# succinctlabs/sp1

Hardware: NVIDIA H100
Metric: riscv_cycles_proven_per_second_core (higher is better)
Workload: dtype u32 KoalaBear (Montgomery) / ext4

## Files before the change

### include/sp1b200.h

```cpp
#ifndef SP1B200_H
#define SP1B200_H
#include <stdint.h>
#include <stddef.h>

#ifdef __cplusplus
extern "C" {
#endif

typedef struct sp1b200_ctx sp1b200_ctx;
typedef const char* sp1b200_err;

typedef struct sp1b200_params {
    uint32_t log_stacking_height;
    uint32_t max_log_row_count;
    uint32_t log_blowup;
    uint32_t num_queries;
    uint32_t pow_bits;
    uint32_t batch_pow_bits;
    uint32_t gkr_pow_bits;
    uint32_t grind_mode;
} sp1b200_params;

#define SP1B200_CHALLENGER_WORDS 34
#define SP1B200_DIGEST_WORDS 8

sp1b200_err sp1b200_ctx_create(int device, const sp1b200_params* params, sp1b200_ctx** out);
void sp1b200_ctx_destroy(sp1b200_ctx* ctx);
sp1b200_err sp1b200_ctx_sync(sp1b200_ctx* ctx);
void sp1b200_default_core_params(sp1b200_params* out);
const char* sp1b200_version(void);
void* sp1b200_ctx_stream(sp1b200_ctx* ctx);
sp1b200_err sp1b200_malloc(sp1b200_ctx* ctx, size_t bytes, void** d_out);
sp1b200_err sp1b200_free(sp1b200_ctx* ctx, void* d_ptr);
sp1b200_err sp1b200_memcpy_h2d(sp1b200_ctx* ctx, void* d_dst, const void* h_src, size_t bytes);
sp1b200_err sp1b200_memcpy_d2h(sp1b200_ctx* ctx, void* h_dst, const void* d_src, size_t bytes);
sp1b200_err sp1b200_pack_row_major(sp1b200_ctx* ctx, const uint32_t* rows_any, uint32_t n_tables, const uint64_t* rows,
                                   const uint64_t* cols, uint32_t* d_dense_out);
sp1b200_err sp1b200_upload_begin(sp1b200_ctx* ctx, const uint32_t* h_src, uint64_t n_words, int slot, uint32_t** d_out);
uint64_t sp1b200_launch_count(sp1b200_ctx* ctx);
float sp1b200_last_phase_ms(sp1b200_ctx* ctx, const char* phase);


sp1b200_err sp1b200_poseidon2_permute(sp1b200_ctx* ctx, uint32_t* states_any, uint64_t n);

sp1b200_err sp1b200_rs_encode(sp1b200_ctx* ctx, const uint32_t* msg_any, uint64_t ncols, uint32_t log_h,
                              uint32_t log_blowup, uint32_t* out_any);

sp1b200_err sp1b200_merkle_commit(sp1b200_ctx* ctx, const uint32_t* mat_any, uint64_t width, uint32_t log_h,
                                  uint32_t* d_layers_out, uint32_t* h_root8, uint32_t* h_commit8);

sp1b200_err sp1b200_grind(sp1b200_ctx* ctx, uint32_t* h_state34, uint32_t bits, uint32_t* h_witness);

void sp1b200_challenger_init(uint32_t* h_state34);
void sp1b200_challenger_observe(uint32_t* h_state34, const uint32_t* h_vals, uint64_t n);
void sp1b200_challenger_sample(uint32_t* h_state34, uint32_t* h_out, uint64_t n);
uint32_t sp1b200_challenger_sample_bits(uint32_t* h_state34, uint32_t bits);
int sp1b200_challenger_check_witness(uint32_t* h_state34, uint32_t bits, uint32_t witness);


typedef struct sp1b200_commit sp1b200_commit;

sp1b200_err sp1b200_stacked_commit(sp1b200_ctx* ctx, const uint32_t* dense_any, uint64_t ncols, int keep_codeword,
                                   uint32_t* h_commit8, sp1b200_commit** out);
void sp1b200_commit_free(sp1b200_ctx* ctx, sp1b200_commit* c);

sp1b200_err sp1b200_stacked_prove(sp1b200_ctx* ctx, sp1b200_commit* const* rounds, uint32_t n_rounds,
                                  const uint32_t* h_point, uint32_t n_point, const uint32_t* h_replay_witnesses,
                                  uint32_t* h_challenger34, uint32_t* h_proof, uint64_t proof_cap_words,
                                  uint64_t* h_proof_words);


typedef struct sp1b200_jagged_round sp1b200_jagged_round;

sp1b200_err sp1b200_jagged_commit(sp1b200_ctx* ctx, const uint32_t* dense_any, uint32_t n_tables, const uint64_t* h_rows,
                                  const uint64_t* h_cols, int keep_codeword, uint32_t* h_commit8, sp1b200_jagged_round** out);
void sp1b200_jagged_round_free(sp1b200_ctx* ctx, sp1b200_jagged_round* round);

sp1b200_err sp1b200_jagged_column_claims(sp1b200_ctx* ctx, const sp1b200_jagged_round* round, const uint32_t* h_z_row,
                                         uint32_t* h_out);

sp1b200_err sp1b200_jagged_prove(sp1b200_ctx* ctx, sp1b200_jagged_round* const* rounds, uint32_t n_rounds,
                                 const uint32_t* h_z_row, const uint32_t* h_claims, const uint32_t* h_replay_witnesses,
                                 uint32_t* h_challenger34, uint32_t* h_proof, uint64_t proof_cap_words,
                                 uint64_t* h_proof_words);


typedef struct sp1b200_machine sp1b200_machine;

sp1b200_err sp1b200_machine_create(sp1b200_ctx* ctx, const uint32_t* h_blob, uint64_t n_words, sp1b200_machine** out);
void sp1b200_machine_free(sp1b200_ctx* ctx, sp1b200_machine* machine);
uint32_t sp1b200_machine_num_chips(const sp1b200_machine* machine);
uint32_t sp1b200_machine_chip_regs(const sp1b200_machine* machine, uint32_t chip);

sp1b200_err sp1b200_zerocheck(sp1b200_ctx* ctx, const sp1b200_machine* machine, const uint64_t* h_heights,
                              const uint32_t* const* d_main, const uint32_t* const* d_prep, const uint32_t* h_public_values,
                              uint32_t n_public_values, const uint32_t* h_gkr_point, const uint32_t* h_alpha,
                              const uint32_t* h_gamma, const uint32_t* h_claims, uint32_t* h_challenger34, uint32_t* h_out,
                              uint64_t out_cap_words, uint64_t* h_out_words);



sp1b200_err sp1b200_logup_gkr(sp1b200_ctx* ctx, const sp1b200_machine* machine, const uint64_t* h_heights,
                              const uint32_t* const* d_main, const uint32_t* const* d_prep, const uint32_t* h_replay_witness,
                              uint32_t* h_challenger34, uint32_t* h_out, uint64_t out_cap_words, uint64_t* h_out_words);


sp1b200_err sp1b200_prove_shard(sp1b200_ctx* ctx, const sp1b200_machine* machine, sp1b200_jagged_round* prep_round,
                                const uint32_t* main_dense_any, const uint64_t* h_heights, const char* const* chip_names,
                                const uint32_t* h_public_values, uint32_t n_public_values, const uint32_t* h_replay_witnesses,
                                uint32_t* h_challenger34, uint32_t* h_proof, uint64_t proof_cap_words, uint64_t* h_proof_words);

sp1b200_err sp1b200_setup_and_prove_shard(sp1b200_ctx* ctx, const sp1b200_machine* machine, const uint32_t* prep_dense_any, uint32_t n_prep,
                                          const uint64_t* h_prep_rows, const uint64_t* h_prep_cols, const uint32_t* h_vk_tail,
                                          uint32_t n_vk_tail, const uint32_t* main_dense_any, const uint64_t* h_heights,
                                          const char* const* chip_names, const uint32_t* h_public_values, uint32_t n_public_values,
                                          const uint32_t* h_replay_witnesses, uint32_t* h_challenger34, uint32_t* h_prep_commit8,
                                          sp1b200_jagged_round** prep_round_out, uint32_t* h_proof, uint64_t proof_cap_words,
                                          uint64_t* h_proof_words);


sp1b200_err sp1b200_debug_constraints(sp1b200_ctx* ctx, const sp1b200_machine* machine, sp1b200_jagged_round* prep_round,
                                      const uint32_t* main_dense_any, const uint64_t* h_heights, const uint32_t* h_public_values,
                                      uint32_t n_public_values, uint32_t max_rows_per_chip, uint32_t* h_out, uint64_t out_cap_words,
                                      uint64_t* h_out_words);

sp1b200_err sp1b200_debug_interactions(sp1b200_ctx* ctx, const sp1b200_machine* machine, sp1b200_jagged_round* prep_round,
                                       const uint32_t* main_dense_any, const uint64_t* h_heights, uint32_t max_keys, uint32_t* h_out,
                                       uint64_t out_cap_words, uint64_t* h_out_words);


sp1b200_err sp1b200_shard_proof_to_bincode(const sp1b200_params* params, uint32_t n_chips, const char* const* chip_names,
                                           const uint64_t* h_heights, const uint32_t* h_main_w, const uint32_t* h_prep_w,
                                           const uint32_t* h_proof, uint64_t n_words, uint8_t* h_out, uint64_t cap_bytes,
                                           uint64_t* h_out_bytes);
sp1b200_err sp1b200_shard_proof_from_bincode(const sp1b200_params* params, uint32_t n_chips, const char* const* chip_names,
                                             const uint32_t* h_main_w, const uint32_t* h_prep_w, const uint8_t* h_bytes, uint64_t n_bytes,
                                             uint64_t* h_heights_out, uint32_t* h_proof, uint64_t cap_words, uint64_t* h_words);

#define SP1B200_VERDICT_ACCEPT 0u
#define SP1B200_VERDICT_POW 1u
#define SP1B200_VERDICT_INVALID_SHAPE 2u
#define SP1B200_VERDICT_ZERO_DENOMINATOR 3u
#define SP1B200_VERDICT_CUMULATIVE_SUM_MISMATCH 4u
#define SP1B200_VERDICT_INVALID_SHAPE_ROUNDS 5u
#define SP1B200_VERDICT_INCONSISTENT_SUMCHECK_CLAIM 6u
#define SP1B200_VERDICT_SUMCHECK_PROOF_SHAPE 7u
#define SP1B200_VERDICT_SUMCHECK_CLAIMED_SUM 8u
#define SP1B200_VERDICT_SUMCHECK_ROUND 9u
#define SP1B200_VERDICT_SUMCHECK_POINT 10u
#define SP1B200_VERDICT_SUMCHECK_EVAL 11u
#define SP1B200_VERDICT_INCONSISTENT_EVALUATION 12u
#define SP1B200_VERDICT_LAST_LAYER_DIMENSION 13u
#define SP1B200_VERDICT_TRACE_POINT_MISMATCH 14u
#define SP1B200_VERDICT_INVALID_SHAPE_OPENINGS 15u
#define SP1B200_VERDICT_NUMERATOR_EVALUATION 16u
#define SP1B200_VERDICT_DENOMINATOR_EVALUATION 17u
#define SP1B200_VERDICT_OPENING_SHAPE 18u
#define SP1B200_VERDICT_HEIGHT_BITS 19u
#define SP1B200_VERDICT_HEIGHT_TOO_LARGE 20u
#define SP1B200_VERDICT_CONSTRAINTS_EVAL 21u
#define SP1B200_VERDICT_CONSTRAINTS_CLAIMED_SUM 22u
#define SP1B200_VERDICT_INCORRECT_SHAPE 23u
#define SP1B200_VERDICT_INCORRECT_TABLE_SIZES 24u
#define SP1B200_VERDICT_AREA_OUT_OF_BOUNDS 25u
#define SP1B200_VERDICT_DUMMY_TABLES 26u
#define SP1B200_VERDICT_SUMCHECK_CLAIM_MISMATCH 27u
#define SP1B200_VERDICT_MONOTONICITY 28u
#define SP1B200_VERDICT_JAGGED_EVALUATION 29u
#define SP1B200_VERDICT_JAGGED_EVAL_PROOF 30u
#define SP1B200_VERDICT_STACKING 31u
#define SP1B200_VERDICT_BATCH_POW 32u
#define SP1B200_VERDICT_FRI_LENGTH 33u
#define SP1B200_VERDICT_BASEFOLD_SUMCHECK 34u
#define SP1B200_VERDICT_TWO_ADICITY 35u
#define SP1B200_VERDICT_TCS_COMPONENT 36u
#define SP1B200_VERDICT_QUERY_VALUE 37u
#define SP1B200_VERDICT_TCS_QUERY 38u
#define SP1B200_VERDICT_QUERY_FINAL_POLY 39u
#define SP1B200_VERDICT_SUMCHECK_FINAL_POLY 40u
#define SP1B200_VERDICT_PREPROCESSED_WIDTHS 41u
#define SP1B200_VERDICT_CHIP_TABLES 42u
sp1b200_err sp1b200_verify_shard(sp1b200_ctx* ctx, const sp1b200_machine* machine, const uint32_t* h_prep_commit8,
                                 const uint64_t* h_heights, const char* const* chip_names, const uint32_t* h_proof, uint64_t n_words,
                                 uint32_t* h_challenger34, uint32_t* h_verdict);
const char* sp1b200_verdict_name(uint32_t verdict);

#define SP1B200_VERDICT_EMPTY_PROOF 43u
#define SP1B200_VERDICT_TOO_MANY_SHARDS 44u
#define SP1B200_VERDICT_INVALID_SHARD_PROOF 45u
#define SP1B200_VERDICT_PV_LENGTH 46u
#define SP1B200_VERDICT_PV_FIRST_SHARD_MULTIPLE 47u
#define SP1B200_VERDICT_PV_FIRST_SHARD_NOT_BOOLEAN 48u
#define SP1B200_VERDICT_PV_FIRST_SHARD_NOT_SET 49u
#define SP1B200_VERDICT_PV_INITIAL_TIMESTAMP 50u
#define SP1B200_VERDICT_PV_TIMESTAMP_UNCHANGED 51u
#define SP1B200_VERDICT_PV_TIMESTAMP_CHANGED 52u
#define SP1B200_VERDICT_PV_PC_START_VK 53u
#define SP1B200_VERDICT_PV_PC_START_PREV 54u
#define SP1B200_VERDICT_PV_PC_NON_EXECUTION 55u
#define SP1B200_VERDICT_PV_NOT_HALTED 56u
#define SP1B200_VERDICT_PV_PREV_EXIT_CODE 57u
#define SP1B200_VERDICT_PV_EXIT_CODE_NON_EXECUTION 58u
#define SP1B200_VERDICT_PV_EXIT_CODE_CHANGED 59u
#define SP1B200_VERDICT_PV_PROOF_NONCE 60u
#define SP1B200_VERDICT_PV_INIT_ADDR 61u
#define SP1B200_VERDICT_PV_FINALIZE_ADDR 62u
#define SP1B200_VERDICT_PV_INIT_PAGE_IDX 63u
#define SP1B200_VERDICT_PV_FINALIZE_PAGE_IDX 64u
#define SP1B200_VERDICT_PV_UNTRUSTED_PROGRAMS 65u
#define SP1B200_VERDICT_PV_NEVER_INITIALIZED 66u
#define SP1B200_VERDICT_PV_NEVER_FINALIZED 67u
#define SP1B200_VERDICT_PV_COMMITTED_VALUE_DIGEST 68u
#define SP1B200_VERDICT_PV_DEFERRED_PROOFS_DIGEST 69u
#define SP1B200_VERDICT_PV_COMMIT_SYSCALL 70u
#define SP1B200_VERDICT_PV_COMMIT_DEFERRED_SYSCALL 71u
#define SP1B200_VERDICT_PV_COMMIT_NEVER_CALLED 72u
#define SP1B200_VERDICT_PV_COMMIT_DEFERRED_NEVER_CALLED 73u
#define SP1B200_VERDICT_PV_GLOBAL_CUMULATIVE_SUM 74u
#define SP1B200_VERDICT_PV_EXCEPTIONAL_ADDITION 75u
#define SP1B200_VERDICT_CORE_COUNT 76u
sp1b200_err sp1b200_verify_core_proof(sp1b200_ctx* ctx, const sp1b200_machine* machine, const uint32_t* h_prep_commit8,
                                      const uint32_t* h_vk_tail, uint32_t n_vk_tail, uint32_t n_shards, const uint64_t* h_heights,
                                      const char* const* chip_names, const uint32_t* const* h_proofs, const uint64_t* h_n_words,
                                      uint32_t host_threads, uint32_t* h_final_challengers, uint32_t* h_verdict, uint32_t* h_shard,
                                      uint32_t* h_shard_verdict);

#ifdef __cplusplus
}
#endif
#endif
```

### sp1_b200/csrc/ctx.cuh

```cuda
#pragma once
#include <cuda_runtime.h>
#include <chrono>
#include <cstdint>
#include <cstdio>
#include <map>
#include <memory>
#include <string>
#include <vector>
#include "../../include/sp1b200.h"

struct sp1b200_ctx {
    int device = 0;
    int num_sms = 132;
    cudaStream_t stream = nullptr;
    cudaMemPool_t pool = nullptr;
    sp1b200_params params{};
    uint32_t* d_TH = nullptr;
    uint32_t* d_TL = nullptr;
    uint32_t* d_T8 = nullptr;
    uint64_t launches = 0;
    bool force_generic_ntt = false;
    std::map<std::string, float> phase_ms;
    cudaEvent_t ev0 = nullptr, ev1 = nullptr;
    uint32_t* h_mail = nullptr;
    uint32_t* d_mail = nullptr;
    uint32_t* d_mail_counter = nullptr;
    uint32_t mail_seq = 0;
    cudaStream_t copy_stream = nullptr;
    uint32_t* d_slot[2] = {nullptr, nullptr};
    uint64_t slot_words[2] = {0, 0};
    cudaEvent_t slot_ready[2] = {nullptr, nullptr};
    cudaEvent_t slot_free[2] = {nullptr, nullptr};
    bool slot_pending[2] = {false, false};
    std::unique_ptr<uint32_t[]> shard_scratch;
};
constexpr size_t SP1_MAIL_HDR = 16;
constexpr size_t SP1_MAIL_WORDS = 1 << 16;

struct Mail { uint32_t* flag; uint32_t* counter; uint32_t seq; };
inline Mail sp1b200_mail_next(sp1b200_ctx* c) { return Mail{c->d_mail, c->d_mail_counter, ++c->mail_seq}; }
inline uint32_t* sp1b200_mail_dev(sp1b200_ctx* c) { return c->d_mail + SP1_MAIL_HDR; }
inline const uint32_t* sp1b200_mail_host(sp1b200_ctx* c) { return c->h_mail + SP1_MAIL_HDR; }
extern "C" sp1b200_err sp1b200_mail_wait(sp1b200_ctx* c, uint32_t seq);

sp1b200_err sp1b200_init_tables(sp1b200_ctx* ctx);
sp1b200_err sp1b200_rs_encode_device(sp1b200_ctx* ctx, const uint32_t* d_msg, uint64_t ncols, uint32_t log_h, uint32_t log_blowup,
                                     uint32_t* d_out);
sp1b200_err sp1b200_permute_device(sp1b200_ctx* ctx, uint32_t* d_states, uint64_t n);
sp1b200_err sp1b200_merkle_commit_device(sp1b200_ctx* ctx, const uint32_t* d_mat, uint64_t width, uint32_t log_h, uint32_t* d_layers,
                                         uint32_t* d_root_commit16);
sp1b200_err sp1b200_merkle_tree_from_leaves_device(sp1b200_ctx* ctx, uint32_t* d_layers, uint32_t log_h, uint32_t width,
                                                   uint32_t* d_root_commit16);
sp1b200_err sp1b200_fri_tree_device(sp1b200_ctx* ctx, const uint32_t* d_cw, uint64_t m, uint32_t* d_layers, uint32_t log_leaves,
                                    uint32_t* d_root_commit16, Mail mail);

#ifdef __CUDACC__
__device__ __forceinline__ void sp1_mail_done(const Mail& m) {
    if (!m.flag) return;
    __threadfence_system();
    __syncthreads();
    if (threadIdx.x == 0 && threadIdx.y == 0 && threadIdx.z == 0) {
        const unsigned total = gridDim.x * gridDim.y * gridDim.z;
        const unsigned prev = atomicAdd(m.counter, 1u);
        if (prev == total - 1) {
            *m.counter = 0;
            __threadfence_system();
            *reinterpret_cast<volatile uint32_t*>(m.flag) = m.seq;
        }
    }
}
#endif

const char* sp1b200_set_error(const char* fmt, ...);
const char* sp1b200_last_error();

struct Sp1DeviceGuard {
    int prev = -1;
    bool switched = false;
    explicit Sp1DeviceGuard(int dev) {
        if (dev < 0) return;
        if (cudaGetDevice(&prev) == cudaSuccess && prev != dev) switched = cudaSetDevice(dev) == cudaSuccess;
    }
    ~Sp1DeviceGuard() { if (switched) cudaSetDevice(prev); }
    Sp1DeviceGuard(const Sp1DeviceGuard&) = delete;
    Sp1DeviceGuard& operator=(const Sp1DeviceGuard&) = delete;
};
#define SP1_DEVICE_GUARD(c) Sp1DeviceGuard _sp1_device_guard((c) ? (c)->device : -1)

#define SP1_CUDA(call)                                                                            \
    do {                                                                                          \
        cudaError_t _e = (call);                                                                  \
        if (_e != cudaSuccess)                                                                    \
            return sp1b200_set_error("%s:%d: %s: %s", __FILE__, __LINE__, #call, cudaGetErrorString(_e)); \
    } while (0)

#define SP1_TRY(call)                   \
    do {                                \
        sp1b200_err _m = (call);        \
        if (_m) return _m;              \
    } while (0)

#define SP1_LAUNCH(ctx, kernel, grid, block, smem, ...)                        \
    do {                                                                       \
        kernel<<<(grid), (block), (smem), (ctx)->stream>>>(__VA_ARGS__);       \
        (ctx)->launches++;                                                     \
        SP1_CUDA(cudaGetLastError());                                          \
    } while (0)

struct PhaseTimer {
    sp1b200_ctx* ctx;
    const char* name;
    cudaEvent_t e0 = nullptr, e1 = nullptr;
    bool done = false;
    PhaseTimer(sp1b200_ctx* c, const char* n) : ctx(c), name(n) {
        cudaEventCreate(&e0); cudaEventCreate(&e1);
        cudaEventRecord(e0, c->stream);
    }
    void stop() {
        if (done) return;
        done = true;
        cudaEventRecord(e1, ctx->stream);
        cudaEventSynchronize(e1);
        float ms = 0;
        cudaEventElapsedTime(&ms, e0, e1);
        ctx->phase_ms[name] = ms;
    }
    ~PhaseTimer() { cudaEventDestroy(e0); cudaEventDestroy(e1); }
};

struct HostAccum {
    sp1b200_ctx* ctx; const char* name; double ms = 0;
    HostAccum(sp1b200_ctx* c, const char* n) : ctx(c), name(n) {}
    ~HostAccum() { ctx->phase_ms[name] = (float)ms; }
};
struct HostSpan {
    HostAccum& a; std::chrono::steady_clock::time_point t0;
    explicit HostSpan(HostAccum& acc) : a(acc), t0(std::chrono::steady_clock::now()) {}
    ~HostSpan() { a.ms += std::chrono::duration<double, std::milli>(std::chrono::steady_clock::now() - t0).count(); }
};

struct DevBuf {
    sp1b200_ctx* ctx = nullptr;
    void* d = nullptr;
    void* host = nullptr;
    size_t bytes = 0;
    bool owned = false;
    sp1b200_err in(sp1b200_ctx* c, const void* any, size_t nbytes);
    sp1b200_err out(sp1b200_ctx* c, void* any, size_t nbytes);
    sp1b200_err finish();
    ~DevBuf();
};

bool sp1b200_is_device_ptr(const void* p);
extern "C" int sp1b200_upload_acquire(sp1b200_ctx* c, const void* d_ptr);
extern "C" void sp1b200_upload_release(sp1b200_ctx* c, int slot);
```

### sp1_b200/csrc/hostcheck.cu

```cuda
#include "poseidon2.cuh"
#include "rs_twiddles.cuh"
#include "debug_fp.cuh"
#include "hostfield.hpp"
#include "septic.hpp"
#include "zc_lower.hpp"
#include <cstring>
#include <type_traits>

extern "C" {
void sp1b200_hostcheck_permute(uint32_t* states, uint64_t n) {
    for (uint64_t i = 0; i < n; i++) {
        uint32_t s[16];
        for (int k = 0; k < 16; k++) s[k] = states[i * 16 + k];
        p2::permute(s);
        for (int k = 0; k < 16; k++) states[i * 16 + k] = s[k];
    }
}
int sp1b200_hostcheck_permute_mode(uint32_t* states, uint64_t n, int mode) {
    for (uint64_t i = 0; i < n; i++) {
        uint32_t s[16];
        for (int k = 0; k < 16; k++) s[k] = states[i * 16 + k];
        switch (mode) {
#define P2_CASE(M) case M: p2::permute_m<M>(s); break;
            P2_CASE(0) P2_CASE(1) P2_CASE(2) P2_CASE(3) P2_CASE(4) P2_CASE(5) P2_CASE(6) P2_CASE(7)
            P2_CASE(8) P2_CASE(9) P2_CASE(10) P2_CASE(11) P2_CASE(12) P2_CASE(13) P2_CASE(14) P2_CASE(15)
            P2_CASE(19) P2_CASE(21) P2_CASE(23)
#undef P2_CASE
            case -1: p2::permute_r1(s); break;
            default: return 0;
        }
        for (int k = 0; k < 16; k++) states[i * 16 + k] = s[k];
    }
    return 1;
}
void sp1b200_hostcheck_ext_mul(const uint32_t* a, const uint32_t* b, uint32_t* out, uint64_t n) {
    for (uint64_t i = 0; i < n; i++) {
        kb::Ext x{{a[4 * i], a[4 * i + 1], a[4 * i + 2], a[4 * i + 3]}}, y{{b[4 * i], b[4 * i + 1], b[4 * i + 2], b[4 * i + 3]}};
        kb::Ext r = kb::ext_mul(x, y);
        for (int k = 0; k < 4; k++) out[4 * i + k] = r.c[k];
    }
}
void sp1b200_hostcheck_ext_inv(const uint32_t* a, uint32_t* out, uint64_t n) {
    for (uint64_t i = 0; i < n; i++) {
        kb::Ext x{{a[4 * i], a[4 * i + 1], a[4 * i + 2], a[4 * i + 3]}};
        kb::Ext r = kb::ext_inv(x);
        for (int k = 0; k < 4; k++) out[4 * i + k] = r.c[k];
    }
}
uint32_t sp1b200_hostcheck_rs_tw8(uint32_t* out) {
    for (uint32_t i = 0; i < rs_tw::WORDS; i++) out[i] = rs_tw::word(i / 8, (int)(i % 8));
    return rs_tw::WORDS;
}
void sp1b200_hostcheck_field(const uint32_t* a, const uint32_t* b, uint32_t* add, uint32_t* sub, uint32_t* mul, uint64_t n) {
    for (uint64_t i = 0; i < n; i++) { add[i] = kb::add(a[i], b[i]); sub[i] = kb::sub(a[i], b[i]); mul[i] = kb::mul(a[i], b[i]); }
}

int sp1b200_hostcheck_zc_lower(const uint32_t* chip, const uint32_t* main_row, const uint32_t* prep_row, const uint32_t* pv,
                               const uint32_t* alpha_pows, uint32_t window, uint32_t* out, uint32_t* n_lowered) {
    using hf::E4;
    const uint32_t* b = chip;
    HostProg hp;
    b += 3;
    const uint32_t n_regs = *b++;
    const uint32_t ni = *b++, nl = *b++, nc = *b++, np = *b++, na = *b++;
    hp.instrs.resize(ni); memcpy(hp.instrs.data(), b, ni * 8); b += 2 * ni;
    hp.leaves.resize(nl); memcpy(hp.leaves.data(), b, nl * 8); b += 2 * nl;
    hp.consts.assign(b, b + nc); b += nc;
    hp.publics.assign(b, b + np); b += np;
    hp.assert_regs.assign(b, b + na); b += na;
    hp.assert_alphas.assign(b, b + na); b += na;
    auto leaf = [&](const LeafRef& l) { return l.source == LEAF_MAIN ? main_row[l.col] : prep_row[l.col]; };
    {
        std::vector<uint32_t> regs(n_regs ? n_regs : 1, 0);
        for (const DagInstr& in : hp.instrs) {
            switch (in.opcode) {
                case BC_LOAD_LEAF: regs[in.out] = leaf(hp.leaves[in.a]); break;
                case BC_LOAD_CONST: regs[in.out] = hp.consts[in.a]; break;
                case BC_LOAD_PUBLIC: regs[in.out] = pv[hp.publics[in.a]]; break;
                case BC_ADD_F: regs[in.out] = hf::add(regs[in.a], regs[in.b]); break;
                case BC_SUB_F: regs[in.out] = hf::sub(regs[in.a], regs[in.b]); break;
                case BC_MUL_F: regs[in.out] = hf::mul(regs[in.a], regs[in.b]); break;
                case BC_NEG_F: regs[in.out] = hf::neg(regs[in.a]); break;
            }
        }
        E4 acc;
        for (size_t k = 0; k < hp.assert_regs.size(); k++) acc = acc + E4::load(alpha_pows + 4 * hp.assert_alphas[k]) * regs[hp.assert_regs[k]];
        acc.store(out);
    }
    auto run = [&](const ZcLowered& Lw) {
        std::vector<uint32_t> rf(Lw.n_regs, 0);
        E4 a;
        for (const ZcInstr& in : Lw.instrs) {
            switch (in.op) {
                case ZC_LOAD_MAIN: rf[in.out] = main_row[(uint32_t)in.a | ((uint32_t)in.b << 16)]; break;
                case ZC_LOAD_PREP: rf[in.out] = prep_row[(uint32_t)in.a | ((uint32_t)in.b << 16)]; break;
                case ZC_CONST: rf[in.out] = hp.consts[in.a]; break;
                case ZC_PUBLIC: rf[in.out] = pv[hp.publics[in.a]]; break;
                case ZC_ADD: { uint32_t x = rf[in.a], y = rf[in.b]; rf[in.out] = hf::add(x, y); break; }
                case ZC_SUB: { uint32_t x = rf[in.a], y = rf[in.b]; rf[in.out] = hf::sub(x, y); break; }
                case ZC_MUL: { uint32_t x = rf[in.a], y = rf[in.b]; rf[in.out] = hf::mul(x, y); break; }
                case ZC_NEG: rf[in.out] = hf::neg(rf[in.a]); break;
                case ZC_ASSERT: a = a + E4::load(alpha_pows + 4 * in.b) * rf[in.a]; break;
            }
        }
        return a;
    };
    ZcLowered L = zc_lower(hp, window);
    if (!L.error.empty()) return -1;
    if (n_lowered) *n_lowered = (uint32_t)L.instrs.size();
    E4 acc = run(L);
    {
        const size_t na = hp.assert_regs.size();
        const size_t np_ = std::max<size_t>(1, std::min<size_t>(16, na / 4));
        E4 sum;
        for (size_t q = 0; q < np_; q++) {
            ZcLowered P = zc_lower(hp, window, na * q / np_, na * (q + 1) / np_);
            if (!P.error.empty() || P.n_regs > L.n_regs + 8) return -1;
            sum = sum + run(P);
        }
        sum.store(out + 8);
    }
    acc.store(out + 4);
    return (int)L.n_regs;
}

uint64_t sp1b200_hostcheck_fingerprint(uint32_t kind, uint32_t n_values, const uint32_t* values) {
    return dbgfp::fingerprint(kind, n_values, values);
}

void sp1b200_hostcheck_e4(const uint32_t* a, const uint32_t* b, uint32_t* mul_out, uint32_t* inv_out, uint64_t n) {
    using hf::E4;
    for (uint64_t i = 0; i < n; i++) {
        (E4::load(a + 4 * i) * E4::load(b + 4 * i)).store(mul_out + 4 * i);
        hf::inv(E4::load(a + 4 * i)).store(inv_out + 4 * i);
    }
}
int sp1b200_hostcheck_interpolate(const uint32_t* xs, const uint32_t* ys, uint32_t n, uint32_t* coeffs_out) {
    using hf::E4;
    auto go = [&](auto tag) {
        constexpr int N = decltype(tag)::value;
        E4 x[N], L[N][N], c[N];
        for (int i = 0; i < N; i++) x[i] = E4::load(xs + 4 * i);
        hf::lagrange_basis<N>(x, L);
        for (int k = 0; k < N; k++) for (int i = 0; i < N; i++) c[k] = c[k] + L[i][k] * E4::load(ys + 4 * i);
        for (int k = 0; k < N; k++) c[k].store(coeffs_out + 4 * k);
    };
    if (n == 3) go(std::integral_constant<int, 3>{});
    else if (n == 4) go(std::integral_constant<int, 4>{});
    else if (n == 5) go(std::integral_constant<int, 5>{});
    else return -1;
    return 0;
}

void sp1b200_hostcheck_septic(const uint32_t* a, const uint32_t* b, uint32_t* mul_out, uint32_t* inv_out, uint64_t n) {
    for (uint64_t i = 0; i < n; i++) {
        const sep::E7 x = sep::E7::load(a + 7 * i), y = sep::E7::load(b + 7 * i);
        (x * y).store(mul_out + 7 * i);
        sep::inv(x).store(inv_out + 7 * i);
    }
}
void sp1b200_hostcheck_septic_curve_add(const uint32_t* p, const uint32_t* q, uint32_t* out, uint32_t* ok, uint64_t n) {
    for (uint64_t i = 0; i < n; i++) {
        const sep::Point a{sep::E7::load(p + 14 * i), sep::E7::load(p + 14 * i + 7)}, b{sep::E7::load(q + 14 * i), sep::E7::load(q + 14 * i + 7)};
        sep::Point r{};
        ok[i] = sep::add_incomplete(a, b, r);
        r.x.store(out + 14 * i); r.y.store(out + 14 * i + 7);
    }
}
int sp1b200_hostcheck_septic_digest_add(const uint32_t* a, const uint32_t* b, uint32_t* out) {
    const sep::Point x{sep::E7::load(a), sep::E7::load(a + 7)}, y{sep::E7::load(b), sep::E7::load(b + 7)};
    sep::Point r{};
    if (!sep::digest_add(x, y, r)) return 0;
    r.x.store(out); r.y.store(out + 7);
    return 1;
}
void sp1b200_hostcheck_septic_constants(uint32_t* out42) {
    const sep::Point pts[3] = {sep::digest_zero(), sep::digest_start(), sep::dummy_point()};
    for (int i = 0; i < 3; i++) { pts[i].x.store(out42 + 14 * i); pts[i].y.store(out42 + 14 * i + 7); }
}
}
```

### sp1_b200/csrc/machine.cuh

```cuda
#pragma once
#include "hostfield.hpp"
#include <algorithm>
#include <cstdint>
#include <type_traits>
#include <utility>
#include <vector>

struct DagInstr { uint8_t opcode, pad; uint16_t out, a, b; };
struct LeafRef { uint8_t source, pad; uint16_t pad2; uint32_t col; };
static_assert(sizeof(DagInstr) == 8 && sizeof(LeafRef) == 8, "bytecode layout must match sequential.cuh");
enum : uint8_t { BC_LOAD_LEAF = 0, BC_LOAD_CONST = 1, BC_LOAD_PUBLIC = 2, BC_ADD_F = 3, BC_SUB_F = 4, BC_MUL_F = 5, BC_NEG_F = 6 };
enum : uint8_t { LEAF_PREP = 2, LEAF_MAIN = 4 };

struct ZcInstr;
struct ChipProg {
    const DagInstr* instrs; const LeafRef* leaves; const uint32_t* consts; const uint32_t* publics;
    const uint32_t* assert_regs; const uint32_t* assert_alphas;
    uint32_t n_instrs, n_asserts, n_regs, main_w, prep_w, n_constraints;
    const ZcInstr* zc; uint32_t n_zc, zc_regs;
};
struct HostProg {
    std::vector<DagInstr> instrs; std::vector<LeafRef> leaves; std::vector<uint32_t> consts, publics, assert_regs, assert_alphas;
    std::vector<std::pair<uint32_t, uint32_t>> zc_pieces;
};

template <class R, class Leaf>
hf::E4 host_eval_constraints(const HostProg& p, uint32_t n_regs, const uint32_t* pv, const std::vector<hf::E4>& powers, Leaf leaf) {
    const auto base = [](uint32_t x) { if constexpr (std::is_same<R, hf::E4>::value) return hf::E4::from_base(x); else return x; };
    std::vector<R> regs(std::max<uint32_t>(n_regs, 1));
    for (const DagInstr& in : p.instrs) {
        switch (in.opcode) {
            case BC_LOAD_LEAF: regs[in.out] = leaf(p.leaves[in.a]); break;
            case BC_LOAD_CONST: regs[in.out] = base(p.consts[in.a]); break;
            case BC_LOAD_PUBLIC: regs[in.out] = base(pv[p.publics[in.a]]); break;
            case BC_ADD_F: regs[in.out] = hf::add(regs[in.a], regs[in.b]); break;
            case BC_SUB_F: regs[in.out] = hf::sub(regs[in.a], regs[in.b]); break;
            case BC_MUL_F: regs[in.out] = hf::mul(regs[in.a], regs[in.b]); break;
            case BC_NEG_F: regs[in.out] = hf::neg(regs[in.a]); break;
        }
    }
    hf::E4 acc;
    for (size_t i = 0; i < p.assert_regs.size(); i++) acc = acc + powers[p.assert_alphas[i]] * regs[p.assert_regs[i]];
    return acc;
}

struct TermDev { uint32_t source, col, weight; };
struct VColDev { uint32_t term_start, n_terms, constant; };
struct InterDev { uint32_t is_send, arg_index, n_values, vcol_start; };
struct HostInteractions {
    std::vector<std::vector<InterDev>> per_chip;
    std::vector<VColDev> vcols;
    std::vector<TermDev> terms;
};

void sp1b200_free_interactions(void* p);

struct sp1b200_machine {
    sp1b200_machine() = default;
    sp1b200_machine(const sp1b200_machine&) = delete;
    sp1b200_machine& operator=(const sp1b200_machine&) = delete;
    ~sp1b200_machine();
    std::vector<ChipProg> chips;
    std::vector<HostProg> host;
    uint32_t* d_arena = nullptr;
    void* d_zc_arena = nullptr;
    ChipProg* d_chips = nullptr;
    void* interactions = nullptr;
};

void* sp1b200_parse_interactions(const uint32_t* b, const uint32_t* end, size_t n_chips, const uint32_t* widths);

typedef const char* sp1b200_err;
struct sp1b200_ctx;
sp1b200_err sp1b200_debug_constraints_device(sp1b200_ctx* ctx, const sp1b200_machine* m, const uint64_t* h_heights, const uint32_t* const* d_main,
                                             const uint32_t* const* d_prep, const uint32_t* h_pv, uint32_t n_pv, uint32_t max_rows,
                                             std::vector<uint32_t>& words);
sp1b200_err sp1b200_debug_interactions_device(sp1b200_ctx* ctx, const sp1b200_machine* m, const uint64_t* h_heights, const uint32_t* const* d_main,
                                              const uint32_t* const* d_prep, uint32_t max_keys, std::vector<uint32_t>& words);
```

### sp1_b200/csrc/zerocheck.cu

```cuda
#include "ctx.cuh"
#include "challenger.cuh"
#include "hostfield.hpp"
#include "kb31.cuh"
#include <algorithm>
#include <memory>
#include <vector>

#include "machine.cuh"
#include "zc_lower.hpp"
#include "sumcheck.cuh"

namespace {

using kb::Ext;
using hf::E4;

constexpr int ZC_BLOCK = 128;
constexpr int ZC_LOCAL_REGS = 128;
constexpr int ZC_GLOBAL_REGS = 1024;
constexpr unsigned ZC_GLOBAL_MAXB = 132 * 2;
constexpr size_t ZC_MAX_PIECES = 16;

inline int zc_tier(uint32_t regs) {
    constexpr uint32_t TIER_REGS[3] = {8, 16, 32};
    for (int t = 0; t < 3; t++) if (regs <= TIER_REGS[t]) return t;
    return regs <= (uint32_t)ZC_LOCAL_REGS ? 3 : 4;
}

template <class K> struct Ops;
template <> struct Ops<uint32_t> {
    static __device__ __forceinline__ uint32_t zero() { return 0; }
    static __device__ __forceinline__ uint32_t from_base(uint32_t x) { return x; }
    static __device__ __forceinline__ uint32_t add(uint32_t a, uint32_t b) { return kb::add(a, b); }
    static __device__ __forceinline__ uint32_t sub(uint32_t a, uint32_t b) { return kb::sub(a, b); }
    static __device__ __forceinline__ uint32_t mul(uint32_t a, uint32_t b) { return kb::mul(a, b); }
    static __device__ __forceinline__ uint32_t load(const uint32_t* p, uint64_t i) { return __ldg(p + i); }
    static __device__ __forceinline__ Ext scale(const Ext& e, uint32_t k) { return kb::ext_mul_base(e, k); }
};
template <> struct Ops<Ext> {
    static __device__ __forceinline__ Ext zero() { return kb::ext_zero(); }
    static __device__ __forceinline__ Ext from_base(uint32_t x) { return kb::ext_from_base(x); }
    static __device__ __forceinline__ Ext add(const Ext& a, const Ext& b) { return kb::ext_add(a, b); }
    static __device__ __forceinline__ Ext sub(const Ext& a, const Ext& b) { return kb::ext_sub(a, b); }
    static __device__ __forceinline__ Ext mul(const Ext& a, const Ext& b) { return kb::ext_mul(a, b); }
    static __device__ __forceinline__ Ext load(const Ext* p, uint64_t i) { return kb::ext_load(reinterpret_cast<const uint32_t*>(p + i)); }
    static __device__ __forceinline__ Ext scale(const Ext& e, const Ext& k) { return kb::ext_mul(e, k); }
};

struct ZcJob {
    const void* main; const void* prep; const uint32_t* alpha_pows; uint64_t h;
    uint32_t blk_start, nblk, chip, columns;
    uint32_t zc_begin, zc_end;
    const void* batch;
};
static_assert(sizeof(ZcJob) == 64, "ZcJob layout");
struct ZcFixJob {
    const void* main; const void* prep; uint32_t* out; uint64_t h;
    uint32_t main_w, prep_w, blk_start, pad;
};

template <class J>
__device__ __forceinline__ int find_job(const J* __restrict__ jobs, int n, uint32_t blk) {
    int lo = 0, hi = n - 1;
    while (lo < hi) {
        int mid = (lo + hi + 1) >> 1;
        if (jobs[mid].blk_start <= blk) lo = mid; else hi = mid - 1;
    }
    return lo;
}

enum { RF_SMEM = 0, RF_LOCAL = 1, RF_GLOBAL = 2 };
template <class K, int RF, int NODES = 3> struct RegFile;
template <class K, int NODES> struct RegFile<K, RF_SMEM, NODES> {
    K* base;
    __device__ __forceinline__ RegFile(unsigned char* smem, void*, uint32_t) : base(reinterpret_cast<K*>(smem) + threadIdx.x) {}
    __device__ __forceinline__ K get(uint32_t r, int n) const { return base[(r * NODES + n) * ZC_BLOCK]; }
    __device__ __forceinline__ void set(uint32_t r, int n, const K& v) { base[(r * NODES + n) * ZC_BLOCK] = v; }
};
template <class K, int NODES> struct RegFile<K, RF_LOCAL, NODES> {
    K regs[ZC_LOCAL_REGS * NODES];
    __device__ __forceinline__ RegFile(unsigned char*, void*, uint32_t) {}
    __device__ __forceinline__ K get(uint32_t r, int n) const { return regs[r * NODES + n]; }
    __device__ __forceinline__ void set(uint32_t r, int n, const K& v) { regs[r * NODES + n] = v; }
};
template <class K, int NODES> struct RegFile<K, RF_GLOBAL, NODES> {
    K* base;
    __device__ __forceinline__ RegFile(unsigned char*, void* ws, uint32_t ws_regs)
        : base(static_cast<K*>(ws) + (size_t)blockIdx.x * ws_regs * NODES * ZC_BLOCK + threadIdx.x) {}
    __device__ __forceinline__ K get(uint32_t r, int n) const { return base[(size_t)(r * NODES + n) * ZC_BLOCK]; }
    __device__ __forceinline__ void set(uint32_t r, int n, const K& v) { base[(size_t)(r * NODES + n) * ZC_BLOCK] = v; }
};

template <class K, int N0>
__device__ __forceinline__ void load_nodes(const K* __restrict__ base, uint32_t col, uint64_t h, uint64_t i, K (&v)[3]) {
    using O = Ops<K>;
    const K* c = base + (uint64_t)col * h;
    const K z = O::load(c, 2 * i);
    const K o = (2 * i + 1 < h) ? O::load(c, 2 * i + 1) : O::zero();
    const K d = O::sub(o, z);
    const K d2 = O::add(d, d);
    if (N0 == 0) v[0] = z;
    v[1] = O::add(z, d2);
    v[2] = O::add(v[1], d2);
}

template <class K, int RF, bool FIRST>
__global__ void __launch_bounds__(ZC_BLOCK) zc_sum_kernel(const ZcJob* __restrict__ jobs, int n_jobs, const ChipProg* __restrict__ chips,
                                                          const uint32_t* __restrict__ pv, const uint32_t* __restrict__ gkr_pows,
                                                          const uint32_t* __restrict__ E, uint32_t* __restrict__ partial,
                                                          void* __restrict__ ws, uint32_t ws_regs) {
    using O = Ops<K>;
    constexpr int N0 = FIRST ? 1 : 0;
    extern __shared__ __align__(16) unsigned char zc_smem[];
    __shared__ uint32_t red[5][4][ZC_BLOCK / 32];
    const ZcJob job = jobs[find_job(jobs, n_jobs, blockIdx.x)];
    const ChipProg& prog = chips[job.chip];
    const K* main = static_cast<const K*>(job.main);
    const K* prep = static_cast<const K*>(job.prep);
    const uint64_t h = job.h;
    const uint64_t terms = (h + 1) / 2;
    RegFile<K, RF> rf(zc_smem, ws, ws_regs);
    Ext acc[5];
#pragma unroll
    for (int a = 0; a < 5; a++) acc[a] = kb::ext_zero();
    const ZcInstr* __restrict__ zc = prog.zc + job.zc_begin;
    const uint32_t n_zc = job.zc_end - job.zc_begin;
    for (uint64_t i = (uint64_t)(blockIdx.x - job.blk_start) * ZC_BLOCK + threadIdx.x; i < terms; i += (uint64_t)job.nblk * ZC_BLOCK) {
        const Ext e = kb::ext_load(E + 4 * i);
        Ext row[3] = {kb::ext_zero(), kb::ext_zero(), kb::ext_zero()};
        ZcInstr in = n_zc ? zc[0] : ZcInstr{};
        for (uint32_t pc = 0; pc < n_zc; pc++) {
            const ZcInstr nxt = zc[pc + 1 < n_zc ? pc + 1 : pc];
            switch (in.op) {
                case ZC_LOAD_MAIN: case ZC_LOAD_PREP: {
                    K v[3];
                    load_nodes<K, N0>(in.op == ZC_LOAD_MAIN ? main : prep, (uint32_t)in.a | ((uint32_t)in.b << 16), h, i, v);
#pragma unroll
                    for (int n = N0; n < 3; n++) rf.set(in.out, n, v[n]);
                    break;
                }
                case ZC_CONST: { const K c = O::from_base(prog.consts[in.a]);
#pragma unroll
                    for (int n = N0; n < 3; n++) rf.set(in.out, n, c);
                    break; }
                case ZC_PUBLIC: { const K c = O::from_base(pv[prog.publics[in.a]]);
#pragma unroll
                    for (int n = N0; n < 3; n++) rf.set(in.out, n, c);
                    break; }
                case ZC_ADD: {
                    K r[3];
#pragma unroll
                    for (int n = N0; n < 3; n++) r[n] = O::add(rf.get(in.a, n), rf.get(in.b, n));
#pragma unroll
                    for (int n = N0; n < 3; n++) rf.set(in.out, n, r[n]);
                    break; }
                case ZC_SUB: {
                    K r[3];
#pragma unroll
                    for (int n = N0; n < 3; n++) r[n] = O::sub(rf.get(in.a, n), rf.get(in.b, n));
#pragma unroll
                    for (int n = N0; n < 3; n++) rf.set(in.out, n, r[n]);
                    break; }
                case ZC_MUL: {
                    K r[3];
#pragma unroll
                    for (int n = N0; n < 3; n++) r[n] = O::mul(rf.get(in.a, n), rf.get(in.b, n));
#pragma unroll
                    for (int n = N0; n < 3; n++) rf.set(in.out, n, r[n]);
                    break; }
                case ZC_NEG: {
                    K r[3];
#pragma unroll
                    for (int n = N0; n < 3; n++) r[n] = O::sub(O::zero(), rf.get(in.a, n));
#pragma unroll
                    for (int n = N0; n < 3; n++) rf.set(in.out, n, r[n]);
                    break; }
                case ZC_ASSERT: {
                    const Ext al = kb::ext_load(job.alpha_pows + 4 * in.b);
#pragma unroll
                    for (int n = N0; n < 3; n++) row[n] = kb::ext_add(row[n], O::scale(al, rf.get(in.a, n)));
                    break; }
                default: __trap();
            }
            in = nxt;
        }
#pragma unroll
        for (int n = N0; n < 3; n++) acc[n] = kb::ext_add(acc[n], kb::ext_mul(row[n], e));
        if (!job.columns) continue;
        Ext s0 = kb::ext_zero(), s1 = kb::ext_zero();
        const bool has_o = 2 * i + 1 < h;
        if (job.batch) {
            const uint32_t* B = static_cast<const uint32_t*>(job.batch);
            acc[3] = kb::ext_add(acc[3], kb::ext_mul(kb::ext_load(B + 8 * i), e));
            if (has_o) acc[4] = kb::ext_add(acc[4], kb::ext_mul(kb::ext_load(B + 8 * i + 4), e));
            continue;
        }
        for (uint32_t j = 0; j < prog.main_w; j++) {
            const Ext g = kb::ext_load(gkr_pows + 4 * j);
            const K* c = main + (uint64_t)j * h;
            s0 = kb::ext_add(s0, O::scale(g, O::load(c, 2 * i)));
            if (has_o) s1 = kb::ext_add(s1, O::scale(g, O::load(c, 2 * i + 1)));
        }
        for (uint32_t j = 0; j < prog.prep_w; j++) {
            const Ext g = kb::ext_load(gkr_pows + 4 * (prog.main_w + j));
            const K* c = prep + (uint64_t)j * h;
            s0 = kb::ext_add(s0, O::scale(g, O::load(c, 2 * i)));
            if (has_o) s1 = kb::ext_add(s1, O::scale(g, O::load(c, 2 * i + 1)));
        }
        acc[3] = kb::ext_add(acc[3], kb::ext_mul(s0, e));
        acc[4] = kb::ext_add(acc[4], kb::ext_mul(s1, e));
    }
    const int lane = threadIdx.x & 31, warp = threadIdx.x >> 5;
#pragma unroll
    for (int a = 0; a < 5; a++)
#pragma unroll
        for (int l = 0; l < 4; l++) {
            uint32_t v = acc[a].c[l];
            for (int s = 16; s > 0; s >>= 1) v = kb::add(v, __shfl_down_sync(0xffffffffu, v, s));
            if (lane == 0) red[a][l][warp] = v;
        }
    __syncthreads();
    if (threadIdx.x < 36) {
        const int node = threadIdx.x / 12, slot = (threadIdx.x >> 2) % 3, l = threadIdx.x & 3;
        const int a = slot == 0 ? node : (node == 0 ? 2 + slot : -1);
        uint32_t v = 0;
        if (a >= 0)
            for (int w = 0; w < ZC_BLOCK / 32; w++) v = kb::add(v, red[a][l][w]);
        partial[(uint64_t)blockIdx.x * 36 + threadIdx.x] = v;
    }
}

__global__ void __launch_bounds__(128) zc_reduce_kernel(const ZcJob* __restrict__ jobs, const uint32_t* __restrict__ partial, uint32_t* __restrict__ out,
                                                        Mail mail) {
    const ZcJob job = jobs[blockIdx.x];
    __shared__ uint32_t red[36][4];
    const int slot = threadIdx.x >> 2, part = threadIdx.x & 3;
    for (int w = slot; w < 36; w += 32) {
        uint32_t v = 0;
        for (uint32_t b = part; b < job.nblk; b += 4) v = kb::add(v, partial[(uint64_t)(job.blk_start + b) * 36 + w]);
        red[w][part] = v;
    }
    __syncthreads();
    if (threadIdx.x < 36) {
        const uint32_t* r = red[threadIdx.x];
        out[blockIdx.x * 36 + threadIdx.x] = kb::add(kb::add(r[0], r[1]), kb::add(r[2], r[3]));
    }
    sp1_mail_done(mail);
}

template <class K>
__global__ void __launch_bounds__(256) zc_fix_kernel(const ZcFixJob* __restrict__ jobs, int n_jobs, Ext alpha) {
    using O = Ops<K>;
    const ZcFixJob job = jobs[find_job(jobs, n_jobs, blockIdx.x)];
    const uint64_t h = job.h, nh = (h + 1) / 2;
    const uint32_t bpc = (uint32_t)((nh + 255) / 256);
    const uint32_t lb = blockIdx.x - job.blk_start;
    const uint64_t j = lb / bpc;
    const uint64_t i = (uint64_t)(lb - (uint32_t)j * bpc) * 256 + threadIdx.x;
    if (i >= nh) return;
    const uint64_t t = j * nh + i;
    const K* in = j < job.main_w ? static_cast<const K*>(job.main) + j * h : static_cast<const K*>(job.prep) + (j - job.main_w) * h;
    K a = O::load(in, 2 * i);
    K b = (2 * i + 1 < h) ? O::load(in, 2 * i + 1) : O::zero();
    Ext r;
    if constexpr (sizeof(K) == 4) r = kb::ext_add(kb::ext_from_base(a), kb::ext_mul_base(alpha, kb::sub(b, a)));
    else r = kb::ext_add(a, kb::ext_mul(alpha, kb::ext_sub(b, a)));
    kb::ext_store(job.out + 4 * t, r);
}

__global__ void __launch_bounds__(256) zc_batch0_kernel(const ZcFixJob* __restrict__ jobs, int n_jobs, const uint32_t* __restrict__ gkr_pows, Ext alpha) {
    const ZcFixJob job = jobs[find_job(jobs, n_jobs, blockIdx.x)];
    const uint64_t h = job.h, nh = (h + 1) / 2;
    const uint64_t i = (uint64_t)(blockIdx.x - job.blk_start) * 256 + threadIdx.x;
    if (i >= nh) return;
    const bool has_o = 2 * i + 1 < h;
    Ext sa = kb::ext_zero(), sd = kb::ext_zero();
    const uint32_t* main = static_cast<const uint32_t*>(job.main);
    const uint32_t* prep = static_cast<const uint32_t*>(job.prep);
    for (uint32_t j = 0; j < job.main_w + job.prep_w; j++) {
        const uint32_t* c = j < job.main_w ? main + (uint64_t)j * h : prep + (uint64_t)(j - job.main_w) * h;
        const uint32_t a = __ldg(c + 2 * i), b = has_o ? __ldg(c + 2 * i + 1) : 0u;
        const Ext g = kb::ext_load(gkr_pows + 4 * j);
        sa = kb::ext_add(sa, kb::ext_mul_base(g, a));
        sd = kb::ext_add(sd, kb::ext_mul_base(g, kb::sub(b, a)));
    }
    kb::ext_store(job.out + 4 * i, kb::ext_add(sa, kb::ext_mul(alpha, sd)));
}

struct ZcDbgJob {
    const uint32_t* main; const uint32_t* prep; uint64_t h;
    const uint32_t* rows;
    uint32_t* out;
    uint32_t* count;
    uint32_t n, blk_start, nblk, chip, cwords, pad;
};
static_assert(sizeof(ZcDbgJob) == 72, "ZcDbgJob layout");

template <int RF, bool LISTED>
__global__ void __launch_bounds__(ZC_BLOCK) zc_debug_kernel(const ZcDbgJob* __restrict__ jobs, int n_jobs, const ChipProg* __restrict__ chips,
                                                            const uint32_t* __restrict__ pv, void* __restrict__ ws, uint32_t ws_regs) {
    extern __shared__ __align__(16) unsigned char zc_smem[];
    const ZcDbgJob job = jobs[find_job(jobs, n_jobs, blockIdx.x)];
    const ChipProg& prog = chips[job.chip];
    RegFile<uint32_t, RF, 1> rf(zc_smem, ws, ws_regs);
    const ZcInstr* __restrict__ zc = prog.zc;
    const uint32_t n_zc = prog.n_zc, lane = threadIdx.x & 31;
    for (uint64_t t0 = (uint64_t)(blockIdx.x - job.blk_start) * ZC_BLOCK + (threadIdx.x - lane); t0 < job.n; t0 += (uint64_t)job.nblk * ZC_BLOCK) {
        const uint64_t t = t0 + lane;
        bool fail = false;
        if (t < job.n) {
            const uint64_t row = LISTED ? job.rows[t] : t;
            for (uint32_t pc = 0; pc < n_zc; pc++) {
                const ZcInstr in = zc[pc];
                switch (in.op) {
                    case ZC_LOAD_MAIN: rf.set(in.out, 0, __ldg(job.main + (uint64_t)((uint32_t)in.a | ((uint32_t)in.b << 16)) * job.h + row)); break;
                    case ZC_LOAD_PREP: rf.set(in.out, 0, __ldg(job.prep + (uint64_t)((uint32_t)in.a | ((uint32_t)in.b << 16)) * job.h + row)); break;
                    case ZC_CONST: rf.set(in.out, 0, prog.consts[in.a]); break;
                    case ZC_PUBLIC: rf.set(in.out, 0, pv[prog.publics[in.a]]); break;
                    case ZC_ADD: rf.set(in.out, 0, kb::add(rf.get(in.a, 0), rf.get(in.b, 0))); break;
                    case ZC_SUB: rf.set(in.out, 0, kb::sub(rf.get(in.a, 0), rf.get(in.b, 0))); break;
                    case ZC_MUL: rf.set(in.out, 0, kb::mul(rf.get(in.a, 0), rf.get(in.b, 0))); break;
                    case ZC_NEG: rf.set(in.out, 0, kb::neg(rf.get(in.a, 0))); break;
                    case ZC_ASSERT:
                        if (rf.get(in.a, 0)) {
                            fail = true;
                            if (LISTED) job.out[t * job.cwords + (in.b >> 5)] |= 1u << (in.b & 31);
                        }
                        break;
                    default: __trap();
                }
            }
        }
        if (!LISTED) {
            const uint32_t bits = __ballot_sync(0xffffffffu, fail);
            if (lane == 0 && bits) { job.out[t0 >> 5] = bits; atomicAdd(job.count, (uint32_t)__popc(bits)); }
        }
    }
}

struct ZcDbgSelect { const uint32_t* bits; uint32_t* rows; uint32_t n_words, take; };
__global__ void __launch_bounds__(32) zc_debug_select_kernel(const ZcDbgSelect* __restrict__ jobs) {
    const ZcDbgSelect s = jobs[blockIdx.x];
    const uint32_t lane = threadIdx.x;
    uint32_t taken = 0;
    for (uint32_t w0 = 0; w0 < s.n_words && taken < s.take; w0 += 32) {
        uint32_t word = w0 + lane < s.n_words ? s.bits[w0 + lane] : 0u;
        const uint32_t c = __popc(word);
        uint32_t incl = c;
        for (int d = 1; d < 32; d <<= 1) {
            const uint32_t x = __shfl_up_sync(0xffffffffu, incl, d);
            if (lane >= (uint32_t)d) incl += x;
        }
        for (uint32_t rank = taken + incl - c; word && rank < s.take; rank++, word &= word - 1)
            s.rows[rank] = (w0 + lane) * 32 + (uint32_t)(__ffs(word) - 1);
        taken += __shfl_sync(0xffffffffu, incl, 31);
    }
}

struct VGeq {
    uint32_t threshold = 0; E4 geq_c, eq_c;
    VGeq fix_last(const E4& a) const {
        VGeq r; r.threshold = threshold >> 1; r.geq_c = geq_c;
        r.eq_c = (threshold & 1) == 0 ? (E4::one() - a) * eq_c : a * (eq_c + geq_c) - geq_c;
        return r;
    }
    E4 at(uint64_t idx) const { return idx < threshold ? E4() : (idx == threshold ? eq_c + geq_c : geq_c); }
};

}

sp1b200_machine::~sp1b200_machine() {
    if (interactions) sp1b200_free_interactions(interactions);
    cudaFree(d_arena);
    cudaFree(d_zc_arena);
    cudaFree(d_chips);
}

extern "C" {

sp1b200_err sp1b200_machine_create(sp1b200_ctx* ctx, const uint32_t* h_blob, uint64_t n_words, sp1b200_machine** out) { SP1_DEVICE_GUARD(ctx);
    auto m = std::make_unique<sp1b200_machine>();
    SP1_CUDA(cudaMalloc((void**)&m->d_arena, n_words * 4 + 16));
    SP1_CUDA(cudaMemcpyAsync(m->d_arena, h_blob, n_words * 4, cudaMemcpyHostToDevice, ctx->stream));
    const uint32_t* b = h_blob;
    const uint32_t* end = h_blob + n_words;
    auto dev = [&](const uint32_t* hp) { return m->d_arena + (hp - h_blob); };
    if (n_words < 1 || !h_blob) return sp1b200_set_error("machine_create: empty blob");
    uint32_t n = *b++;
    for (uint32_t c = 0; c < n; c++) {
        if ((uint64_t)(end - b) < 9) return sp1b200_set_error("machine_create: truncated blob (header of chip %u)", c);
        ChipProg p{}; HostProg hp;
        p.main_w = *b++; p.prep_w = *b++; p.n_constraints = *b++; p.n_regs = *b++;
        const uint64_t ni = *b++, nl = *b++, nc = *b++, np = *b++, na = *b++;
        if (2 * ni + 2 * nl + nc + np + 2 * na > (uint64_t)(end - b)) return sp1b200_set_error("machine_create: truncated blob (chip %u)", c);
        if (p.n_regs > 65536) return sp1b200_set_error("machine_create: chip %u declares %u registers (16-bit register indices)", c, p.n_regs);
        p.n_instrs = (uint32_t)ni; p.n_asserts = (uint32_t)na;
        p.instrs = reinterpret_cast<const DagInstr*>(dev(b)); hp.instrs.resize(ni); memcpy(hp.instrs.data(), b, ni * 8); b += 2 * ni;
        p.leaves = reinterpret_cast<const LeafRef*>(dev(b)); hp.leaves.resize(nl); memcpy(hp.leaves.data(), b, nl * 8); b += 2 * nl;
        p.consts = dev(b); hp.consts.assign(b, b + nc); b += nc;
        p.publics = dev(b); hp.publics.assign(b, b + np); b += np;
        p.assert_regs = dev(b); hp.assert_regs.assign(b, b + na); b += na;
        p.assert_alphas = dev(b); hp.assert_alphas.assign(b, b + na); b += na;
        for (const LeafRef& l : hp.leaves) {
            if (l.source != LEAF_MAIN && l.source != LEAF_PREP) return sp1b200_set_error("machine_create: chip %u: leaf source %u (expected 2 = preprocessed or 4 = main)", c, l.source);
            if (l.col >= (l.source == LEAF_MAIN ? p.main_w : p.prep_w)) return sp1b200_set_error("machine_create: chip %u: leaf column %u outside the %s width", c, l.col, l.source == LEAF_MAIN ? "main" : "preprocessed");
        }
        for (size_t k = 0; k < hp.instrs.size(); k++) {
            const DagInstr& in = hp.instrs[k];
            if (in.out >= p.n_regs) return sp1b200_set_error("machine_create: chip %u instr %zu: output register %u >= n_regs %u", c, k, in.out, p.n_regs);
            bool ok = true;
            switch (in.opcode) {
                case BC_LOAD_LEAF: ok = in.a < nl; break;
                case BC_LOAD_CONST: ok = in.a < nc; break;
                case BC_LOAD_PUBLIC: ok = in.a < np; break;
                case BC_ADD_F: case BC_SUB_F: case BC_MUL_F: ok = in.a < p.n_regs && in.b < p.n_regs; break;
                case BC_NEG_F: ok = in.a < p.n_regs; break;
                default: return sp1b200_set_error("machine_create: chip %u instr %zu: unknown opcode %u", c, k, in.opcode);
            }
            if (!ok) return sp1b200_set_error("machine_create: chip %u instr %zu: operand out of range (opcode %u, a %u, b %u)", c, k, in.opcode, in.a, in.b);
        }
        for (size_t k = 0; k < hp.assert_regs.size(); k++) {
            if (hp.assert_regs[k] >= p.n_regs) return sp1b200_set_error("machine_create: chip %u assert %zu: register %u >= n_regs %u", c, k, hp.assert_regs[k], p.n_regs);
            if (hp.assert_alphas[k] >= p.n_constraints) return sp1b200_set_error("machine_create: chip %u assert %zu: alpha index %u >= n_constraints %u", c, k, hp.assert_alphas[k], p.n_constraints);
        }
        m->chips.push_back(p); m->host.push_back(std::move(hp));
    }
    {
        std::vector<uint32_t> widths;
        for (auto& c : m->chips) { widths.push_back(c.main_w); widths.push_back(c.prep_w); }
        widths.push_back(0);
        m->interactions = sp1b200_parse_interactions(b, end, n, widths.data());
        if (!m->interactions) return sp1b200_last_error();
    }
    std::vector<ZcInstr> all;
    std::vector<size_t> zc_off(n);
    for (uint32_t c = 0; c < n; c++) {
        ZcLowered L = zc_lower(m->host[c]);
        if (!L.error.empty()) return sp1b200_set_error("machine_create: chip %u: %s", c, L.error.c_str());
        zc_off[c] = all.size();
        m->chips[c].n_zc = (uint32_t)L.instrs.size();
        m->chips[c].zc_regs = L.n_regs;
        all.insert(all.end(), L.instrs.begin(), L.instrs.end());
        const size_t na = m->host[c].assert_regs.size();
        const size_t np_ = std::min<size_t>(ZC_MAX_PIECES, na / 4);
        if (np_ >= 2 && L.instrs.size() >= 128) {
            for (size_t q = 0; q < np_; q++) {
                ZcLowered P = zc_lower(m->host[c], 24, na * q / np_, na * (q + 1) / np_);
                if (!P.error.empty()) return sp1b200_set_error("machine_create: chip %u: %s", c, P.error.c_str());
                m->host[c].zc_pieces.emplace_back((uint32_t)(all.size() - zc_off[c]), (uint32_t)P.instrs.size());
                m->chips[c].zc_regs = std::max(m->chips[c].zc_regs, P.n_regs);
                all.insert(all.end(), P.instrs.begin(), P.instrs.end());
            }
        }
    }
    SP1_CUDA(cudaMalloc(&m->d_zc_arena, all.size() * sizeof(ZcInstr) + 16));
    if (!all.empty()) SP1_CUDA(cudaMemcpyAsync(m->d_zc_arena, all.data(), all.size() * sizeof(ZcInstr), cudaMemcpyHostToDevice, ctx->stream));
    for (uint32_t c = 0; c < n; c++) m->chips[c].zc = static_cast<const ZcInstr*>(m->d_zc_arena) + zc_off[c];
    SP1_CUDA(cudaMalloc((void**)&m->d_chips, (n ? n : 1) * sizeof(ChipProg)));
    if (n) SP1_CUDA(cudaMemcpyAsync(m->d_chips, m->chips.data(), n * sizeof(ChipProg), cudaMemcpyHostToDevice, ctx->stream));
    SP1_CUDA(cudaStreamSynchronize(ctx->stream));
    *out = m.release();
    return nullptr;
}
void sp1b200_machine_free(sp1b200_ctx*, sp1b200_machine* m) { delete m; }
uint32_t sp1b200_machine_chip_regs(const sp1b200_machine* m, uint32_t chip) { return chip < m->chips.size() ? m->chips[chip].zc_regs : 0; }
uint32_t sp1b200_machine_num_chips(const sp1b200_machine* m) { return (uint32_t)m->chips.size(); }

sp1b200_err sp1b200_zerocheck(sp1b200_ctx* ctx, const sp1b200_machine* m, const uint64_t* h_heights, const uint32_t* const* d_main,
                              const uint32_t* const* d_prep, const uint32_t* h_pv, uint32_t n_pv, const uint32_t* h_gkr_point,
                              const uint32_t* h_alpha, const uint32_t* h_gamma, const uint32_t* h_claims, uint32_t* h_chal, uint32_t* h_out,
                              uint64_t cap, uint64_t* h_words) { SP1_DEVICE_GUARD(ctx);
    const uint32_t mlr = ctx->params.max_log_row_count;
    const size_t nchips = m->chips.size();
    for (size_t k = 0; k < nchips; k++)
        for (uint32_t pi : m->host[k].publics)
            if (pi >= n_pv) return sp1b200_set_error("zerocheck: chip %zu reads public value %u but only %u were passed", k, pi, n_pv);
    cudaStream_t st = ctx->stream;
    DevFree mem(ctx);
    HostChallenger ch;
    SP1_TRY(ch.init(ctx, h_chal));
    PhaseTimer t_all(ctx, "zerocheck.total");
    HostAccum acc_wait(ctx, "zerocheck.host_wait"), acc_math(ctx, "zerocheck.host_math"), acc_setup(ctx, "zerocheck.host_setup");
    auto t_setup = std::make_unique<HostSpan>(acc_setup);
    const E4 alpha = E4::load(h_alpha), gamma = E4::load(h_gamma);

    struct St {
        uint64_t h;
        std::vector<E4> zeta; E4 eq_adj = E4::one(), pra; VGeq vg;
    };
    std::vector<St> S(nchips);
    size_t maxc = 0, maxw = 0, total_w = 0, total_c = 0;
    for (auto& c : m->chips) {
        maxc = std::max<size_t>(maxc, c.n_constraints); maxw = std::max<size_t>(maxw, c.main_w + c.prep_w);
        total_w += c.main_w + c.prep_w; total_c += c.n_constraints ? c.n_constraints : 1;
    }
    std::vector<E4> pw(maxc ? maxc : 1); pw[0] = E4::one();
    for (size_t i = 1; i < pw.size(); i++) pw[i] = pw[i - 1] * alpha;
    std::vector<E4> gw(maxw ? maxw : 1); gw[0] = gamma;
    for (size_t i = 1; i < gw.size(); i++) gw[i] = gw[i - 1] * gamma;
    uint32_t *d_pv, *d_gw, *d_ap;
    SP1_TRY(mem.alloc((void**)&d_pv, (n_pv ? n_pv : 1) * 4));
    if (n_pv) SP1_CUDA(cudaMemcpyAsync(d_pv, h_pv, n_pv * 4, cudaMemcpyHostToDevice, st));
    SP1_TRY(mem.alloc((void**)&d_gw, gw.size() * 16));
    SP1_CUDA(cudaMemcpyAsync(d_gw, gw.data(), gw.size() * 16, cudaMemcpyHostToDevice, st));
    std::vector<E4> gp(mlr);
    for (uint32_t i = 0; i < mlr; i++) gp[i] = E4::load(h_gkr_point + 4 * i);
    std::vector<E4> all_ap; all_ap.reserve(total_c);
    std::vector<size_t> ap_off(nchips), woff(nchips);
    std::vector<uint64_t> boff0(nchips), boff1(nchips);
    uint64_t b0 = 0, b1 = 0; size_t wsum = 0;
    for (size_t k = 0; k < nchips; k++) {
        const ChipProg& p = m->chips[k];
        St& s = S[k];
        s.h = h_heights[k];
        if (s.h > ((uint64_t)1 << mlr)) return sp1b200_set_error("zerocheck: chip %zu height exceeds 2^%u", k, mlr);
        if (p.zc_regs > ZC_GLOBAL_REGS) return sp1b200_set_error("zerocheck: chip %zu needs %u live registers (> %d)", k, p.zc_regs, ZC_GLOBAL_REGS);
        s.zeta = gp;
        std::vector<E4> rev(pw.begin(), pw.begin() + p.n_constraints);
        std::reverse(rev.begin(), rev.end());
        ap_off[k] = all_ap.size();
        all_ap.insert(all_ap.end(), rev.begin(), rev.end());
        if (rev.empty()) all_ap.push_back(E4());
        s.pra = host_eval_constraints<uint32_t>(m->host[k], p.n_regs, h_pv, rev, [](const LeafRef&) { return 0u; });
        s.vg.threshold = (uint32_t)s.h; s.vg.geq_c = E4::one();
        const uint64_t nh = (s.h + 1) / 2;
        const size_t w = p.main_w + p.prep_w;
        boff0[k] = b0; b0 += (uint64_t)(w + 1) * nh * 4;
        boff1[k] = b1; b1 += (uint64_t)(w + 1) * ((nh + 1) / 2) * 4;
        woff[k] = wsum; wsum += w;
    }
    SP1_TRY(mem.alloc((void**)&d_ap, all_ap.size() * 16));
    SP1_CUDA(cudaMemcpyAsync(d_ap, all_ap.data(), all_ap.size() * 16, cudaMemcpyHostToDevice, st));
    uint32_t *d_buf[2], *d_final;
    SP1_TRY(mem.alloc((void**)&d_buf[0], b0 * 4 + 16));
    SP1_TRY(mem.alloc((void**)&d_buf[1], b1 * 4 + 16));
    SP1_TRY(mem.alloc((void**)&d_final, (wsum ? wsum : 1) * 16));
    uint32_t *d_point, *d_E[2];
    SP1_TRY(mem.alloc((void**)&d_point, mlr * 16));
    SP1_CUDA(cudaMemcpyAsync(d_point, h_gkr_point, mlr * 16, cudaMemcpyHostToDevice, st));
    SP1_TRY(mem.alloc((void**)&d_E[0], ((size_t)16 << (mlr - 1))));
    SP1_TRY(mem.alloc((void**)&d_E[1], ((size_t)16 << (mlr > 1 ? mlr - 2 : 0))));
    SP1_TRY(launch_eq_table(ctx, d_point, (int)mlr - 1, d_E[0]));
    int ecur = 0;

    size_t ws_bytes = 0;
    struct Launch { size_t job0; uint32_t n_jobs, blocks, regs; int tier; };
    struct RoundPlan { std::vector<Launch> sums; size_t fix0; uint32_t fix_jobs, fix_blocks; std::vector<uint32_t> chip_of_job; size_t job0; };
    std::vector<RoundPlan> plan(mlr);
    std::vector<ZcJob> jobs;
    std::vector<ZcFixJob> fjobs, bjobs;
    uint32_t batch_blocks = 0;
    const unsigned MAXB = 132 * 4;
    uint32_t max_blocks = 1, max_jobs = 1;
    {
        std::vector<uint64_t> hcur(nchips);
        for (size_t k = 0; k < nchips; k++) hcur[k] = S[k].h;
        for (uint32_t rd = 0; rd < mlr; rd++) {
            RoundPlan& R = plan[rd];
            R.job0 = jobs.size();
            auto in_main = [&](size_t k) -> const void* {
                if (rd == 0) return d_main[k];
                return (rd & 1 ? d_buf[0] + boff0[k] : d_buf[1] + boff1[k]);
            };
            auto in_prep = [&](size_t k) -> const void* {
                const ChipProg& p = m->chips[k];
                if (rd == 0) return p.prep_w ? d_prep[k] : nullptr;
                return static_cast<const uint32_t*>(in_main(k)) + (uint64_t)p.main_w * hcur[k] * 4;
            };
            auto in_batch = [&](size_t k) -> const void* {
                if (rd == 0) return nullptr;
                const ChipProg& p = m->chips[k];
                return static_cast<const uint32_t*>(in_main(k)) + (uint64_t)(p.main_w + p.prep_w) * hcur[k] * 4;
            };
            uint32_t blocks_round = 0;
            for (int tier = 0; tier < 5; tier++) {
                Launch Lc{jobs.size(), 0, 0, 0, tier};
                for (size_t k = 0; k < nchips; k++) {
                    const ChipProg& p = m->chips[k];
                    if (!hcur[k] || zc_tier(p.zc_regs) != tier) continue;
                    unsigned nb = blocks_for((hcur[k] + 1) / 2, ZC_BLOCK);
                    if (nb > MAXB) nb = MAXB;
                    if (tier == 4 && nb > ZC_GLOBAL_MAXB) nb = ZC_GLOBAL_MAXB;
                    const auto& pieces = m->host[k].zc_pieces;
                    if (nb <= 16 && !pieces.empty()) {
                        for (size_t q = 0; q < pieces.size(); q++) {
                            ZcJob j{in_main(k), in_prep(k), d_ap + 4 * ap_off[k], hcur[k], Lc.blocks, nb, (uint32_t)k, q == 0 ? 1u : 0u,
                                    pieces[q].first, pieces[q].first + pieces[q].second, in_batch(k)};
                            jobs.push_back(j);
                            R.chip_of_job.push_back((uint32_t)k);
                            Lc.n_jobs++; Lc.blocks += nb;
                        }
                    } else {
                        ZcJob j{in_main(k), in_prep(k), d_ap + 4 * ap_off[k], hcur[k], Lc.blocks, nb, (uint32_t)k, 1u, 0u, p.n_zc, in_batch(k)};
                        jobs.push_back(j);
                        R.chip_of_job.push_back((uint32_t)k);
                        Lc.n_jobs++; Lc.blocks += nb;
                    }
                    Lc.regs = std::max(Lc.regs, p.zc_regs);
                }
                if (Lc.n_jobs) {
                    R.sums.push_back(Lc); blocks_round += Lc.blocks;
                    if (tier == 4) ws_bytes = std::max(ws_bytes, (size_t)Lc.blocks * Lc.regs * 3 * ZC_BLOCK * 16);
                }
            }
            max_blocks = std::max(max_blocks, blocks_round);
            max_jobs = std::max<uint32_t>(max_jobs, (uint32_t)R.chip_of_job.size());
            R.fix0 = fjobs.size(); R.fix_jobs = 0; R.fix_blocks = 0;
            for (size_t k = 0; k < nchips; k++) {
                const ChipProg& p = m->chips[k];
                if (!hcur[k]) continue;
                const uint64_t nh = (hcur[k] + 1) / 2;
                uint32_t* out = rd + 1 == mlr ? d_final + 4 * woff[k] : (rd & 1 ? d_buf[1] + boff1[k] : d_buf[0] + boff0[k]);
                const uint32_t fold_b = (rd > 0 && rd + 1 < mlr) ? 1u : 0u;
                ZcFixJob f{in_main(k), in_prep(k), out, hcur[k], p.main_w, p.prep_w + fold_b, R.fix_blocks, 0};
                fjobs.push_back(f);
                R.fix_jobs++; R.fix_blocks += blocks_for(nh, 256) * (p.main_w + p.prep_w + fold_b);
                if (rd == 0 && mlr > 1) {
                    ZcFixJob bj{d_main[k], m->chips[k].prep_w ? d_prep[k] : nullptr, d_buf[0] + boff0[k] + (uint64_t)(p.main_w + p.prep_w) * nh * 4, hcur[k],
                                p.main_w, p.prep_w, batch_blocks, 0};
                    bjobs.push_back(bj);
                    batch_blocks += blocks_for(nh, 256);
                }
                hcur[k] = nh;
            }
        }
    }
    ZcJob* d_jobs; ZcFixJob *d_fjobs, *d_bjobs; uint32_t *d_partial, *d_sums;
    SP1_TRY(mem.alloc((void**)&d_jobs, (jobs.size() + 1) * sizeof(ZcJob)));
    SP1_TRY(mem.alloc((void**)&d_fjobs, (fjobs.size() + 1) * sizeof(ZcFixJob)));
    SP1_TRY(mem.alloc((void**)&d_bjobs, (bjobs.size() + 1) * sizeof(ZcFixJob)));
    if (!bjobs.empty()) SP1_CUDA(cudaMemcpyAsync(d_bjobs, bjobs.data(), bjobs.size() * sizeof(ZcFixJob), cudaMemcpyHostToDevice, st));
    if (!jobs.empty()) SP1_CUDA(cudaMemcpyAsync(d_jobs, jobs.data(), jobs.size() * sizeof(ZcJob), cudaMemcpyHostToDevice, st));
    if (!fjobs.empty()) SP1_CUDA(cudaMemcpyAsync(d_fjobs, fjobs.data(), fjobs.size() * sizeof(ZcFixJob), cudaMemcpyHostToDevice, st));
    SP1_TRY(mem.alloc((void**)&d_partial, (size_t)max_blocks * 36 * 4));
    if ((size_t)max_jobs * 36 > SP1_MAIL_WORDS) return sp1b200_set_error("zerocheck: %u chips exceed the mailbox payload", max_jobs);
    d_sums = sp1b200_mail_dev(ctx);
    SP1_CUDA(cudaMemsetAsync(d_final, 0, (wsum ? wsum : 1) * 16, st));
    void* d_ws = nullptr;
    if (ws_bytes) SP1_TRY(mem.alloc(&d_ws, ws_bytes));
    auto launch_sum = [&](const Launch& Lc, bool ext, uint32_t* part) -> sp1b200_err {
        auto go = [&](auto kern, size_t smem) -> sp1b200_err {
            if (smem > 32 * 1024) SP1_CUDA(cudaFuncSetAttribute(kern, cudaFuncAttributeMaxDynamicSharedMemorySize, (int)smem));
            SP1_LAUNCH(ctx, kern, Lc.blocks, ZC_BLOCK, smem, d_jobs + Lc.job0, (int)Lc.n_jobs, m->d_chips, d_pv, d_gw, d_E[ecur], part, d_ws,
                       Lc.regs);
            return nullptr;
        };
        if (Lc.tier == 4) return ext ? go(zc_sum_kernel<Ext, RF_GLOBAL, false>, 0) : go(zc_sum_kernel<uint32_t, RF_GLOBAL, true>, 0);
        if (Lc.tier == 3) return ext ? go(zc_sum_kernel<Ext, RF_LOCAL, false>, 0) : go(zc_sum_kernel<uint32_t, RF_LOCAL, true>, 0);
        const size_t regs = Lc.regs;
        return ext ? go(zc_sum_kernel<Ext, RF_SMEM, false>, regs * 3 * ZC_BLOCK * 16) : go(zc_sum_kernel<uint32_t, RF_SMEM, true>, regs * 3 * ZC_BLOCK * 4);
    };

    t_setup.reset();
    E4 lambda; ch.sample_ext(lambda.c);
    std::vector<E4> round_claims(nchips);
    E4 claimed_sum;
    for (size_t k = 0; k < nchips; k++) { round_claims[k] = E4::load(h_claims + 4 * k); claimed_sum = claimed_sum * lambda + round_claims[k]; }
    std::vector<uint32_t> words;
    words.push_back(mlr);
    std::vector<E4> point;
    std::vector<E4> ys((size_t)nchips * 4);
    std::vector<uint32_t> hs((size_t)max_jobs * 36);
    std::vector<E4> chip_sums(nchips * 9);
    const E4 two = E4::from_base(hf::to_monty(2)), four = E4::from_base(hf::to_monty(4)), three = E4::from_base(hf::to_monty(3));
    for (uint32_t rd = 0; rd < mlr; rd++) {
        const RoundPlan& R = plan[rd];
        {
            uint32_t blk = 0, seq = 0; size_t jb = 0;
            for (const Launch& Lc : R.sums) {
                SP1_TRY(launch_sum(Lc, rd > 0, d_partial + (size_t)blk * 36));
                const Mail mail = sp1b200_mail_next(ctx); seq = mail.seq;
                SP1_LAUNCH(ctx, zc_reduce_kernel, Lc.n_jobs, 128, 0, d_jobs + Lc.job0, d_partial + (size_t)blk * 36, d_sums + jb * 36, mail);
                blk += Lc.blocks; jb += Lc.n_jobs;
            }
            if (jb) {
                HostSpan sp(acc_wait);
                SP1_TRY(sp1b200_mail_wait(ctx, seq));
                memcpy(hs.data(), sp1b200_mail_host(ctx), jb * 36 * 4);
            }
        }
        HostSpan sp_math(acc_math);
        std::fill(chip_sums.begin(), chip_sums.end(), E4());
        for (size_t j = 0; j < R.chip_of_job.size(); j++)
            for (int w9 = 0; w9 < 9; w9++) chip_sums[(size_t)R.chip_of_job[j] * 9 + w9] = chip_sums[(size_t)R.chip_of_job[j] * 9 + w9] + E4::load(&hs[j * 36 + 4 * w9]);
        const E4 last = gp[mlr - 1 - rd];
        const E4 bnode = (E4::one() - last) * hf::inv(E4::one() - (last + last));
        const E4 nodes[5] = {E4(), E4::one(), two, four, bnode};
        E4 basis[5][5];
        hf::lagrange_basis<5>(nodes, basis);
        const E4 f0 = E4::one() - last, f2 = last * hf::to_monty(3) - E4::one(), f4 = last * hf::to_monty(7) - three;
        E4 Y[4];
        for (size_t k = 0; k < nchips; k++) {
            St& s = S[k];
            E4* y = &ys[4 * k];
            if (s.h == 0) { y[0] = y[1] = y[2] = y[3] = E4(); }
            else {
                const E4* q = &chip_sums[k * 9];
                const E4 A = q[1], B = q[2];
                E4 y0 = q[0] + A;
                E4 y2 = q[3] + (B + B) - A;
                E4 y4 = q[6] + B * four - A * three;
                const uint64_t th = (s.h + 1) / 2 - 1;
                const uint64_t esize = (uint64_t)1 << (s.zeta.size() - 1);
                E4 eth;
                if (th < esize) {
                    const size_t kk = s.zeta.size() - 1;
                    eth = E4::one();
                    for (size_t t = 0; t < kk; t++) eth = eth * (((th >> (kk - 1 - t)) & 1) ? s.zeta[t] : E4::one() - s.zeta[t]);
                }
                const E4 msb = s.eq_adj * eth;
                const E4 v0 = s.vg.fix_last(E4()).at(th), v2 = s.vg.fix_last(two).at(th), v4 = s.vg.fix_last(four).at(th);
                y0 = y0 * (f0 * s.eq_adj) - s.pra * v0 * msb * f0;
                y2 = y2 * (f2 * s.eq_adj) - s.pra * v2 * msb * f2;
                y4 = y4 * (f4 * s.eq_adj) - s.pra * v4 * msb * f4;
                y[0] = y0; y[1] = round_claims[k] - y0; y[2] = y2; y[3] = y4;
            }
            for (int i = 0; i < 4; i++) Y[i] = (k ? Y[i] * lambda : E4()) + y[i];
        }
        E4 rlc[5];
        for (int c5 = 0; c5 < 5; c5++) for (int i = 0; i < 4; i++) rlc[c5] = rlc[c5] + basis[i][c5] * Y[i];
        for (auto& c : rlc) ch.observe_n(c.c, 4);
        words.push_back(5);
        for (auto& c : rlc) words.insert(words.end(), c.c, c.c + 4);
        E4 a; ch.sample_ext(a.c);
        point.insert(point.begin(), a);
        const Ext da = to_ext(a);
        if (R.fix_jobs) {
            if (rd == 0) {
                SP1_LAUNCH(ctx, zc_fix_kernel<uint32_t>, R.fix_blocks, 256, 0, d_fjobs + R.fix0, (int)R.fix_jobs, da);
                if (!bjobs.empty()) SP1_LAUNCH(ctx, zc_batch0_kernel, batch_blocks, 256, 0, d_bjobs, (int)bjobs.size(), d_gw, da);
            } else SP1_LAUNCH(ctx, zc_fix_kernel<Ext>, R.fix_blocks, 256, 0, d_fjobs + R.fix0, (int)R.fix_jobs, da);
        }
        E4 La[4];
        for (int i = 0; i < 4; i++) La[i] = hf::eval_poly<5>(basis[i], a);
        for (size_t k = 0; k < nchips; k++) {
            St& s = S[k];
            const E4* y = &ys[4 * k];
            round_claims[k] = y[0] * La[0] + y[1] * La[1] + y[2] * La[2] + y[3] * La[3];
            s.vg = s.vg.fix_last(a);
            if (s.h == 0) continue;
            s.eq_adj = s.eq_adj * (a * last + (E4::one() - a) * (E4::one() - last));
            s.zeta.pop_back();
            s.h = (s.h + 1) / 2;
        }
        if (rd + 1 < mlr) {
            const uint64_t n_out = (uint64_t)1 << (mlr - 2 - rd);
            SP1_TRY(launch_halve_eq(ctx, d_E[ecur], n_out, d_E[ecur ^ 1]));
            ecur ^= 1;
        }
    }
    E4 final_eval;
    for (auto& c : round_claims) final_eval = final_eval * lambda + c;
    words.insert(words.end(), claimed_sum.c, claimed_sum.c + 4);
    for (auto& x : point) words.insert(words.end(), x.c, x.c + 4);
    words.insert(words.end(), final_eval.c, final_eval.c + 4);
    std::vector<uint32_t> fin((wsum ? wsum : 1) * 4);
    SP1_CUDA(cudaMemcpyAsync(fin.data(), d_final, fin.size() * 4, cudaMemcpyDeviceToHost, st));
    SP1_CUDA(cudaStreamSynchronize(st));
    ch.observe(hf::to_monty(nchips));
    for (size_t k = 0; k < nchips; k++) {
        const ChipProg& p = m->chips[k];
        const uint32_t* mv = &fin[4 * woff[k]];
        const uint32_t* pvv = mv + 4 * (size_t)p.main_w;
        ch.observe(hf::to_monty(p.prep_w)); ch.observe_n(pvv, (size_t)p.prep_w * 4);
        ch.observe(hf::to_monty(p.main_w)); ch.observe_n(mv, (size_t)p.main_w * 4);
        words.insert(words.end(), pvv, pvv + (size_t)p.prep_w * 4);
        words.insert(words.end(), mv, mv + (size_t)p.main_w * 4);
    }
    t_all.stop();
    ch.store(h_chal);
    if (h_words) *h_words = words.size();
    if (words.size() > cap) return sp1b200_set_error("zerocheck: output needs %zu words, capacity %llu", words.size(), (unsigned long long)cap);
    if (h_out) memcpy(h_out, words.data(), words.size() * 4);
    return nullptr;
}

}

sp1b200_err sp1b200_debug_constraints_device(sp1b200_ctx* ctx, const sp1b200_machine* m, const uint64_t* h_heights, const uint32_t* const* d_main,
                                             const uint32_t* const* d_prep, const uint32_t* h_pv, uint32_t n_pv, uint32_t max_rows,
                                             std::vector<uint32_t>& words) {
    const size_t nchips = m->chips.size();
    for (size_t k = 0; k < nchips; k++) {
        for (uint32_t pi : m->host[k].publics)
            if (pi >= n_pv) return sp1b200_set_error("debug_constraints: chip %zu reads public value %u but only %u were passed", k, pi, n_pv);
        if (m->chips[k].zc_regs > ZC_GLOBAL_REGS)
            return sp1b200_set_error("debug_constraints: chip %zu needs %u live registers (> %d)", k, m->chips[k].zc_regs, ZC_GLOBAL_REGS);
    }
    cudaStream_t st = ctx->stream;
    DevFree mem(ctx);
    PhaseTimer t_all(ctx, "debug_constraints.total");
    uint32_t* d_pv;
    SP1_TRY(mem.alloc((void**)&d_pv, (n_pv ? n_pv : 1) * 4));
    if (n_pv) SP1_CUDA(cudaMemcpyAsync(d_pv, h_pv, n_pv * 4, cudaMemcpyHostToDevice, st));
    struct Launch { size_t job0; uint32_t n_jobs, blocks, regs; int tier; };
    auto plan = [&](std::vector<ZcDbgJob>& jobs, std::vector<Launch>& launches, size_t& ws_bytes, auto n_of, auto fill) {
        for (int tier = 0; tier < 5; tier++) {
            Launch Lc{jobs.size(), 0, 0, 0, tier};
            for (size_t k = 0; k < nchips; k++) {
                const uint64_t n = n_of(k);
                if (!n || zc_tier(m->chips[k].zc_regs) != tier) continue;
                unsigned nb = std::min<unsigned>(blocks_for(n, ZC_BLOCK), 132 * 4);
                if (tier == 4) nb = std::min(nb, ZC_GLOBAL_MAXB);
                ZcDbgJob j{};
                j.main = d_main[k]; j.prep = m->chips[k].prep_w ? d_prep[k] : nullptr; j.h = h_heights[k];
                j.n = (uint32_t)n; j.blk_start = Lc.blocks; j.nblk = nb; j.chip = (uint32_t)k;
                fill(k, j);
                jobs.push_back(j);
                Lc.n_jobs++; Lc.blocks += nb; Lc.regs = std::max(Lc.regs, m->chips[k].zc_regs);
            }
            if (Lc.n_jobs) {
                launches.push_back(Lc);
                if (tier == 4) ws_bytes = std::max(ws_bytes, (size_t)Lc.blocks * Lc.regs * ZC_BLOCK * 4);
            }
        }
    };
    auto run = [&](const std::vector<ZcDbgJob>& jobs, const std::vector<Launch>& launches, size_t ws_bytes, bool listed) -> sp1b200_err {
        ZcDbgJob* d_jobs;
        void* d_ws = nullptr;
        SP1_TRY(mem.alloc((void**)&d_jobs, (jobs.size() + 1) * sizeof(ZcDbgJob)));
        if (!jobs.empty()) SP1_CUDA(cudaMemcpyAsync(d_jobs, jobs.data(), jobs.size() * sizeof(ZcDbgJob), cudaMemcpyHostToDevice, st));
        if (ws_bytes) SP1_TRY(mem.alloc(&d_ws, ws_bytes));
        for (const Launch& Lc : launches) {
            auto go = [&](auto kern, size_t smem) -> sp1b200_err {
                SP1_LAUNCH(ctx, kern, Lc.blocks, ZC_BLOCK, smem, d_jobs + Lc.job0, (int)Lc.n_jobs, m->d_chips, d_pv, d_ws, Lc.regs);
                return nullptr;
            };
            sp1b200_err e;
            if (Lc.tier == 4) e = listed ? go(zc_debug_kernel<RF_GLOBAL, true>, 0) : go(zc_debug_kernel<RF_GLOBAL, false>, 0);
            else if (Lc.tier == 3) e = listed ? go(zc_debug_kernel<RF_LOCAL, true>, 0) : go(zc_debug_kernel<RF_LOCAL, false>, 0);
            else e = listed ? go(zc_debug_kernel<RF_SMEM, true>, (size_t)Lc.regs * ZC_BLOCK * 4)
                            : go(zc_debug_kernel<RF_SMEM, false>, (size_t)Lc.regs * ZC_BLOCK * 4);
            SP1_TRY(e);
        }
        return nullptr;
    };

    std::vector<uint64_t> bm_off(nchips);
    uint64_t bm_words = 0;
    for (size_t k = 0; k < nchips; k++) { bm_off[k] = bm_words; bm_words += (h_heights[k] + 31) / 32; }
    uint32_t *d_bm, *d_cnt;
    SP1_TRY(mem.alloc((void**)&d_bm, (bm_words ? bm_words : 1) * 4));
    SP1_TRY(mem.alloc((void**)&d_cnt, (nchips ? nchips : 1) * 4));
    SP1_CUDA(cudaMemsetAsync(d_bm, 0, (bm_words ? bm_words : 1) * 4, st));
    SP1_CUDA(cudaMemsetAsync(d_cnt, 0, (nchips ? nchips : 1) * 4, st));
    {
        std::vector<ZcDbgJob> jobs; std::vector<Launch> launches; size_t ws = 0;
        plan(jobs, launches, ws, [&](size_t k) { return h_heights[k]; },
             [&](size_t k, ZcDbgJob& j) { j.out = d_bm + bm_off[k]; j.count = d_cnt + k; });
        SP1_TRY(run(jobs, launches, ws, false));
    }
    std::vector<uint32_t> cnt(nchips);
    if (nchips) SP1_CUDA(cudaMemcpyAsync(cnt.data(), d_cnt, nchips * 4, cudaMemcpyDeviceToHost, st));
    SP1_CUDA(cudaStreamSynchronize(st));

    std::vector<uint64_t> row_off(nchips), cbm_off(nchips);
    std::vector<uint32_t> take(nchips), cwords(nchips);
    uint64_t n_rows = 0, n_cbm = 0;
    std::vector<ZcDbgSelect> sel;
    uint32_t* d_rows;
    for (size_t k = 0; k < nchips; k++) {
        take[k] = std::min(cnt[k], max_rows);
        cwords[k] = (m->chips[k].n_constraints + 31) / 32;
        row_off[k] = n_rows; n_rows += take[k];
        cbm_off[k] = n_cbm; n_cbm += (uint64_t)take[k] * cwords[k];
    }
    SP1_TRY(mem.alloc((void**)&d_rows, (n_rows ? n_rows : 1) * 4));
    std::vector<uint32_t> rows(n_rows), cbm(n_cbm);
    if (n_rows) {
        for (size_t k = 0; k < nchips; k++)
            if (take[k]) sel.push_back(ZcDbgSelect{d_bm + bm_off[k], d_rows + row_off[k], (uint32_t)((h_heights[k] + 31) / 32), take[k]});
        ZcDbgSelect* d_sel;
        uint32_t* d_cbm;
        SP1_TRY(mem.alloc((void**)&d_sel, sel.size() * sizeof(ZcDbgSelect)));
        SP1_TRY(mem.alloc((void**)&d_cbm, (n_cbm ? n_cbm : 1) * 4));
        SP1_CUDA(cudaMemcpyAsync(d_sel, sel.data(), sel.size() * sizeof(ZcDbgSelect), cudaMemcpyHostToDevice, st));
        SP1_CUDA(cudaMemsetAsync(d_cbm, 0, (n_cbm ? n_cbm : 1) * 4, st));
        SP1_LAUNCH(ctx, zc_debug_select_kernel, (unsigned)sel.size(), 32, 0, d_sel);
        std::vector<ZcDbgJob> jobs; std::vector<Launch> launches; size_t ws = 0;
        plan(jobs, launches, ws, [&](size_t k) { return (uint64_t)take[k]; },
             [&](size_t k, ZcDbgJob& j) { j.rows = d_rows + row_off[k]; j.out = d_cbm + cbm_off[k]; j.cwords = cwords[k]; });
        SP1_TRY(run(jobs, launches, ws, true));
        SP1_CUDA(cudaMemcpyAsync(rows.data(), d_rows, n_rows * 4, cudaMemcpyDeviceToHost, st));
        if (n_cbm) SP1_CUDA(cudaMemcpyAsync(cbm.data(), d_cbm, n_cbm * 4, cudaMemcpyDeviceToHost, st));
        SP1_CUDA(cudaStreamSynchronize(st));
    }
    t_all.stop();
    words.assign(1, 0);
    for (size_t k = 0; k < nchips; k++) {
        if (!cnt[k]) continue;
        words[0]++;
        words.push_back((uint32_t)k); words.push_back(cnt[k]); words.push_back(take[k]);
        for (uint32_t i = 0; i < take[k]; i++) {
            words.push_back(rows[row_off[k] + i]);
            const size_t n_at = words.size();
            words.push_back(0);
            const uint32_t* b = &cbm[cbm_off[k] + (uint64_t)i * cwords[k]];
            for (uint32_t c = 0; c < m->chips[k].n_constraints; c++)
                if ((b[c >> 5] >> (c & 31)) & 1) { words.push_back(c); words[n_at]++; }
        }
    }
    return nullptr;
}
```

### sp1_b200/lib.py

```python
import ctypes as C
import os

import numpy as np

HERE = os.path.dirname(os.path.abspath(__file__))
SO_PATH = os.path.join(HERE, "libsp1b200.so")

u32p = C.POINTER(C.c_uint32)


PV = dict(prev_committed_value_digest=(0, 32), committed_value_digest=(32, 32), prev_deferred_proofs_digest=(64, 8),
          deferred_proofs_digest=(72, 8), pc_start=(80, 3), next_pc=(83, 3), prev_exit_code=(86, 1), exit_code=(87, 1),
          is_execution_shard=(88, 1), previous_init_addr=(89, 3), last_init_addr=(92, 3), previous_finalize_addr=(95, 3),
          last_finalize_addr=(98, 3), previous_init_page_idx=(101, 3), last_init_page_idx=(104, 3), previous_finalize_page_idx=(107, 3),
          last_finalize_page_idx=(110, 3), initial_timestamp=(113, 4), last_timestamp=(117, 4), is_timestamp_high_eq=(121, 1),
          inv_timestamp_high=(122, 1), is_timestamp_low_eq=(123, 1), inv_timestamp_low=(124, 1), global_init_count=(125, 1),
          global_finalize_count=(126, 1), global_page_prot_init_count=(127, 1), global_page_prot_finalize_count=(128, 1),
          global_count=(129, 1), global_cumulative_sum=(130, 14), prev_commit_syscall=(144, 1), commit_syscall=(145, 1),
          prev_commit_deferred_syscall=(146, 1), commit_deferred_syscall=(147, 1), initial_timestamp_inv=(148, 1),
          last_timestamp_inv=(149, 1), is_first_execution_shard=(150, 1), is_untrusted_programs_enabled=(151, 1), proof_nonce=(152, 4),
          empty=(156, 4))
PV_NUM_ELTS = 160
PV_MAX_NUM = 187
VK_TAIL_WORDS = 24


class Params(C.Structure):
    _fields_ = [(n, C.c_uint32) for n in ("log_stacking_height", "max_log_row_count", "log_blowup", "num_queries",
                                          "pow_bits", "batch_pow_bits", "gkr_pow_bits", "grind_mode")]


DEFAULT_CORE_PARAMS = dict(log_stacking_height=21, max_log_row_count=22, log_blowup=2, num_queries=124, pow_bits=16,
                           batch_pow_bits=5, gkr_pow_bits=12, grind_mode=0)


class Sp1B200Error(RuntimeError):
    pass


_cdll = None


def load():
    global _cdll
    if _cdll is None:
        if not os.path.exists(SO_PATH):
            raise Sp1B200Error(f"{SO_PATH} is missing: run `python -c 'import __graft_entry__ as g; g.build()'` "
                               "(there is no CPU fallback)")
        L = C.CDLL(SO_PATH)
        L.sp1b200_version.restype = C.c_char_p
        L.sp1b200_ctx_stream.restype = C.c_void_p
        L.sp1b200_launch_count.restype = C.c_uint64
        L.sp1b200_last_phase_ms.restype = C.c_float
        L.sp1b200_challenger_sample_bits.restype = C.c_uint32
        L.sp1b200_challenger_check_witness.restype = C.c_int
        L.sp1b200_machine_num_chips.restype = C.c_uint32
        L.sp1b200_machine_chip_regs.restype = C.c_uint32
        L.sp1b200_verdict_name.restype = C.c_char_p
        for name in ERR_FUNCS:
            getattr(L, name).restype = C.c_char_p
        _cdll = L
    return _cdll


ERR_FUNCS = [
    "sp1b200_ctx_create", "sp1b200_ctx_sync", "sp1b200_malloc", "sp1b200_free", "sp1b200_memcpy_h2d",
    "sp1b200_memcpy_d2h", "sp1b200_upload_begin", "sp1b200_pack_row_major", "sp1b200_poseidon2_permute", "sp1b200_rs_encode", "sp1b200_merkle_commit", "sp1b200_grind",
    "sp1b200_stacked_commit", "sp1b200_stacked_prove", "sp1b200_jagged_commit", "sp1b200_jagged_column_claims",
    "sp1b200_jagged_prove", "sp1b200_machine_create", "sp1b200_zerocheck", "sp1b200_logup_gkr", "sp1b200_prove_shard",
    "sp1b200_setup_and_prove_shard", "sp1b200_shard_proof_to_bincode", "sp1b200_shard_proof_from_bincode",
    "sp1b200_debug_constraints", "sp1b200_debug_interactions", "sp1b200_verify_shard", "sp1b200_verify_core_proof",
]
OTHER_FUNCS = ["sp1b200_challenger_init", "sp1b200_challenger_observe", "sp1b200_challenger_sample",
               "sp1b200_challenger_sample_bits", "sp1b200_challenger_check_witness", "sp1b200_ctx_destroy", "sp1b200_default_core_params", "sp1b200_version", "sp1b200_ctx_stream",
               "sp1b200_launch_count", "sp1b200_last_phase_ms", "sp1b200_commit_free", "sp1b200_jagged_round_free",
               "sp1b200_machine_free", "sp1b200_machine_num_chips", "sp1b200_machine_chip_regs",
               "sp1b200_verdict_name"]


def _ptr(a):
    if a is None:
        return None
    if isinstance(a, int):
        return C.c_void_p(a)
    if isinstance(a, np.ndarray):
        assert a.dtype == np.uint32 and a.flags["C_CONTIGUOUS"], "need contiguous uint32"
        return C.c_void_p(a.ctypes.data)
    if hasattr(a, "data_ptr"):
        assert a.is_contiguous() and a.element_size() == 4
        return C.c_void_p(a.data_ptr())
    raise TypeError(type(a))


class Lib:

    def __init__(self, device=0, **params):
        self.L = load()
        p = dict(DEFAULT_CORE_PARAMS)
        p.update(params)
        self.params = p
        self._p = Params(**p)
        self.ctx = C.c_void_p()
        self._chk(self.L.sp1b200_ctx_create(C.c_int(device), C.byref(self._p), C.byref(self.ctx)))

    def _chk(self, err):
        if err:
            raise Sp1B200Error(err.decode())

    def close(self):
        if self.ctx:
            self.L.sp1b200_ctx_destroy(self.ctx)
            self.ctx = C.c_void_p()

    def __del__(self):
        try:
            self.close()
        except Exception:
            pass

    def sync(self):
        self._chk(self.L.sp1b200_ctx_sync(self.ctx))

    def stream(self):
        return self.L.sp1b200_ctx_stream(self.ctx)

    def launch_count(self):
        return int(self.L.sp1b200_launch_count(self.ctx))

    def phase_ms(self, name):
        return float(self.L.sp1b200_last_phase_ms(self.ctx, name.encode()))

    def poseidon2_permute(self, states):
        n = states.shape[0] if hasattr(states, "shape") else None
        self._chk(self.L.sp1b200_poseidon2_permute(self.ctx, _ptr(states), C.c_uint64(n)))
        return states

    def rs_encode(self, msg, out, ncols, log_h, log_blowup=None):
        lb = self.params["log_blowup"] if log_blowup is None else log_blowup
        self._chk(self.L.sp1b200_rs_encode(self.ctx, _ptr(msg), C.c_uint64(ncols), C.c_uint32(log_h), C.c_uint32(lb),
                                           _ptr(out)))
        return out

    def merkle_commit(self, mat, width, log_h, d_layers=None):
        root = np.zeros(8, np.uint32)
        commit = np.zeros(8, np.uint32)
        self._chk(self.L.sp1b200_merkle_commit(self.ctx, _ptr(mat), C.c_uint64(width), C.c_uint32(log_h), _ptr(d_layers),
                                               _ptr(root), _ptr(commit)))
        return root, commit

    def stacked_commit(self, dense, ncols, keep_codeword=True):
        commit = np.zeros(8, np.uint32)
        h = C.c_void_p()
        self._chk(self.L.sp1b200_stacked_commit(self.ctx, _ptr(dense), C.c_uint64(ncols), C.c_int(int(keep_codeword)),
                                                _ptr(commit), C.byref(h)))
        return commit, h

    def commit_free(self, handle):
        self.L.sp1b200_commit_free(self.ctx, handle)

    def stacked_prove(self, handles, point, challenger_state, replay=None, cap_words=1 << 24):
        n = len(handles)
        arr = (C.c_void_p * n)(*[h.value for h in handles])
        point = np.ascontiguousarray(point, dtype=np.uint32)
        proof = np.empty(cap_words, np.uint32)
        nwords = C.c_uint64()
        rw = None if replay is None else np.ascontiguousarray(replay, dtype=np.uint32)
        self._chk(self.L.sp1b200_stacked_prove(self.ctx, arr, C.c_uint32(n), _ptr(point), C.c_uint32(point.shape[0]),
                                               _ptr(rw), _ptr(challenger_state), _ptr(proof), C.c_uint64(cap_words),
                                               C.byref(nwords)))
        return proof[:nwords.value].copy()

    def jagged_commit(self, tables, keep_codeword=True):
        rows = [int(t.shape[1]) for t in tables]
        cols = [int(t.shape[0]) for t in tables]
        parts = [np.ascontiguousarray(t, dtype=np.uint32).reshape(-1) for t in tables if t.shape[1]]
        dense = np.ascontiguousarray(np.concatenate(parts)) if parts else np.zeros(1, np.uint32)
        return self.jagged_commit_dense(dense, rows, cols, keep_codeword)

    def jagged_commit_dense(self, dense, rows, cols, keep_codeword=True):
        n = len(rows)
        R = (C.c_uint64 * n)(*rows)
        Cc = (C.c_uint64 * n)(*cols)
        commit = np.zeros(8, np.uint32)
        h = C.c_void_p()
        self._chk(self.L.sp1b200_jagged_commit(self.ctx, _ptr(dense), C.c_uint32(n), R, Cc, C.c_int(int(keep_codeword)),
                                               _ptr(commit), C.byref(h)))
        return commit, h

    def jagged_round_free(self, handle):
        self.L.sp1b200_jagged_round_free(self.ctx, handle)

    def jagged_column_claims(self, handle, z_row, ncols_total):
        z = np.ascontiguousarray(z_row, dtype=np.uint32)
        out = np.zeros((ncols_total, 4), np.uint32)
        self._chk(self.L.sp1b200_jagged_column_claims(self.ctx, handle, _ptr(z), _ptr(out)))
        return out

    def jagged_prove(self, handles, z_row, claims, challenger_state, replay=None, cap_words=1 << 24):
        n = len(handles)
        arr = (C.c_void_p * n)(*[h.value for h in handles])
        z = np.ascontiguousarray(z_row, dtype=np.uint32)
        cl = np.ascontiguousarray(claims, dtype=np.uint32)
        proof = np.empty(cap_words, np.uint32)
        nwords = C.c_uint64()
        rw = None if replay is None else np.ascontiguousarray(replay, dtype=np.uint32)
        self._chk(self.L.sp1b200_jagged_prove(self.ctx, arr, C.c_uint32(n), _ptr(z), _ptr(cl), _ptr(rw),
                                              _ptr(challenger_state), _ptr(proof), C.c_uint64(cap_words), C.byref(nwords)))
        return proof[:nwords.value].copy()

    def machine_create(self, blob):
        blob = np.ascontiguousarray(blob, dtype=np.uint32)
        h = C.c_void_p()
        self._chk(self.L.sp1b200_machine_create(self.ctx, _ptr(blob), C.c_uint64(blob.size), C.byref(h)))
        return h

    def machine_chip_regs(self, h, chip):
        return int(self.L.sp1b200_machine_chip_regs(h, C.c_uint32(chip)))

    def machine_free(self, h):
        self.L.sp1b200_machine_free(self.ctx, h)

    def zerocheck(self, machine, heights, d_mains, d_preps, pv, gkr_point, alpha, gamma, claims, challenger_state, cap_words=1 << 22):
        n = len(heights)
        H = (C.c_uint64 * n)(*heights)
        M = (C.c_void_p * n)(*[t.data_ptr() if t is not None and t.numel() else None for t in d_mains])
        Pp = (C.c_void_p * n)(*[t.data_ptr() if t is not None and t.numel() else None for t in d_preps])
        pv = np.ascontiguousarray(pv, dtype=np.uint32)
        out = np.empty(cap_words, np.uint32)
        nw = C.c_uint64()
        self._chk(self.L.sp1b200_zerocheck(self.ctx, machine, H, M, Pp, _ptr(pv), C.c_uint32(pv.size),
                                           _ptr(np.ascontiguousarray(gkr_point, dtype=np.uint32)),
                                           _ptr(np.ascontiguousarray(alpha, dtype=np.uint32)),
                                           _ptr(np.ascontiguousarray(gamma, dtype=np.uint32)),
                                           _ptr(np.ascontiguousarray(claims, dtype=np.uint32)), _ptr(challenger_state), _ptr(out),
                                           C.c_uint64(cap_words), C.byref(nw)))
        return out[:nw.value].copy()

    def logup_gkr(self, machine, heights, d_mains, d_preps, challenger_state, replay=None, cap_words=1 << 22):
        n = len(heights)
        H = (C.c_uint64 * n)(*heights)
        M = (C.c_void_p * n)(*[t.data_ptr() if t is not None and t.numel() else None for t in d_mains])
        Pp = (C.c_void_p * n)(*[t.data_ptr() if t is not None and t.numel() else None for t in d_preps])
        out = np.empty(cap_words, np.uint32)
        nw = C.c_uint64()
        rw = None if replay is None else np.ascontiguousarray([replay], dtype=np.uint32)
        self._chk(self.L.sp1b200_logup_gkr(self.ctx, machine, H, M, Pp, _ptr(rw), _ptr(challenger_state), _ptr(out),
                                           C.c_uint64(cap_words), C.byref(nw)))
        return out[:nw.value].copy()

    def prove_shard(self, machine, prep_round, main_dense, heights, names, pv, challenger_state, replay=None, cap_words=1 << 24):
        n = len(heights)
        H = (C.c_uint64 * n)(*heights)
        NM = (C.c_char_p * n)(*[s.encode() for s in names])
        pv = np.ascontiguousarray(pv, dtype=np.uint32)
        out = np.empty(cap_words, np.uint32)
        nw = C.c_uint64()
        rw = None if replay is None else np.ascontiguousarray(replay, dtype=np.uint32)
        self._chk(self.L.sp1b200_prove_shard(self.ctx, machine, prep_round, _ptr(main_dense), H, NM, _ptr(pv), C.c_uint32(pv.size),
                                             _ptr(rw), _ptr(challenger_state), _ptr(out), C.c_uint64(cap_words), C.byref(nw)))
        return out[:nw.value].copy()

    def verify_shard(self, machine, prep_commit, heights, names, words, challenger_state):
        n = len(heights)
        H = (C.c_uint64 * max(1, n))(*heights)
        NM = (C.c_char_p * max(1, n))(*[s.encode() for s in names])
        w = np.ascontiguousarray(words, dtype=np.uint32)
        st = np.ascontiguousarray(challenger_state, dtype=np.uint32).copy()
        pc = None if prep_commit is None else np.ascontiguousarray(prep_commit, dtype=np.uint32)
        verdict = C.c_uint32()
        self._chk(self.L.sp1b200_verify_shard(self.ctx, machine, _ptr(pc), H, NM, _ptr(w), C.c_uint64(w.size), _ptr(st), C.byref(verdict)))
        return int(verdict.value), st

    def verify_core_proof(self, machine, prep_commit, vk_tail, heights_per_shard, names, words_per_shard, host_threads=0):
        n = len(words_per_shard)
        nch = len(names)
        H = np.ascontiguousarray(np.asarray(heights_per_shard, dtype=np.uint64).reshape(n * nch) if n else np.zeros(1, np.uint64))
        NM = (C.c_char_p * max(1, nch))(*[s.encode() for s in names])
        ws = [None if w is None else np.ascontiguousarray(w, dtype=np.uint32) for w in words_per_shard]
        P = (C.c_void_p * max(1, n))(*[None if w is None else w.ctypes.data for w in ws])
        NW = (C.c_uint64 * max(1, n))(*[0 if w is None else w.size for w in ws])
        pc = np.ascontiguousarray(prep_commit, dtype=np.uint32)
        tail = np.ascontiguousarray(vk_tail, dtype=np.uint32)
        fin = np.zeros((max(1, n), 34), np.uint32)
        verdict, shard, sv = C.c_uint32(), C.c_uint32(), C.c_uint32()
        self._chk(self.L.sp1b200_verify_core_proof(self.ctx, machine, _ptr(pc), _ptr(tail), C.c_uint32(tail.size), C.c_uint32(n),
                                                    C.c_void_p(H.ctypes.data), NM, P, NW, C.c_uint32(host_threads), _ptr(fin),
                                                    C.byref(verdict), C.byref(shard), C.byref(sv)))
        v = int(verdict.value)
        return v, int(shard.value), int(sv.value), (fin[:n].copy() if v == 0 else None)

    def _debug_call(self, fn, args, cap_words):
        out = np.empty(max(1, cap_words), np.uint32)
        nw = C.c_uint64()
        self._chk(fn(self.ctx, *args, _ptr(out), C.c_uint64(cap_words), C.byref(nw)))
        return out[:nw.value].copy()

    def debug_constraints_words(self, machine, prep_round, main_dense, heights, pv, max_rows=3, cap_words=1 << 22):
        H = (C.c_uint64 * len(heights))(*heights)
        pv = np.ascontiguousarray(pv, dtype=np.uint32)
        return self._debug_call(self.L.sp1b200_debug_constraints, (machine, prep_round, _ptr(main_dense), H, _ptr(pv), C.c_uint32(pv.size),
                                                                  C.c_uint32(max_rows)), cap_words)

    def debug_interactions_words(self, machine, prep_round, main_dense, heights, max_keys=16, cap_words=1 << 22):
        H = (C.c_uint64 * len(heights))(*heights)
        return self._debug_call(self.L.sp1b200_debug_interactions, (machine, prep_round, _ptr(main_dense), H, C.c_uint32(max_keys)), cap_words)

    def debug_constraints(self, machine, prep_round, main_dense, heights, pv, max_rows=3, cap_words=1 << 22):
        return parse_constraint_report(self.debug_constraints_words(machine, prep_round, main_dense, heights, pv, max_rows, cap_words))

    def debug_interactions(self, machine, prep_round, main_dense, heights, max_keys=16, cap_words=1 << 22):
        return parse_interaction_report(self.debug_interactions_words(machine, prep_round, main_dense, heights, max_keys, cap_words))

    def setup_and_prove_shard(self, machine, prep_dense, prep_rows, prep_cols, vk_tail, main_dense, heights, names, pv, challenger_state,
                              replay=None, cap_words=1 << 24):
        n = len(heights)
        H = (C.c_uint64 * n)(*heights)
        NM = (C.c_char_p * n)(*[s.encode() for s in names])
        npz = len(prep_rows)
        R = (C.c_uint64 * max(1, npz))(*prep_rows)
        Cc = (C.c_uint64 * max(1, npz))(*prep_cols)
        pv = np.ascontiguousarray(pv, dtype=np.uint32)
        tail = np.ascontiguousarray(vk_tail, dtype=np.uint32)
        out = np.empty(cap_words, np.uint32)
        nw = C.c_uint64()
        pc = np.zeros(8, np.uint32)
        h = C.c_void_p()
        rw = None if replay is None else np.ascontiguousarray(replay, dtype=np.uint32)
        self._chk(self.L.sp1b200_setup_and_prove_shard(self.ctx, machine, _ptr(prep_dense), C.c_uint32(npz), R, Cc, _ptr(tail), C.c_uint32(tail.size),
                                                       _ptr(main_dense), H, NM, _ptr(pv), C.c_uint32(pv.size), _ptr(rw), _ptr(challenger_state),
                                                       _ptr(pc), C.byref(h), _ptr(out), C.c_uint64(cap_words), C.byref(nw)))
        return pc, h, out[:nw.value].copy()

    def pack_row_major(self, rows_any, shapes, d_dense_out):
        n = len(shapes)
        R = (C.c_uint64 * n)(*[int(r) for r, _ in shapes])
        Cc = (C.c_uint64 * n)(*[int(c) for _, c in shapes])
        self._chk(self.L.sp1b200_pack_row_major(self.ctx, _ptr(rows_any), C.c_uint32(n), R, Cc, _ptr(d_dense_out)))

    def upload_begin(self, host_array, slot):
        d = C.c_void_p()
        n = host_array.numel() if hasattr(host_array, "numel") else host_array.size
        self._chk(self.L.sp1b200_upload_begin(self.ctx, _ptr(host_array), C.c_uint64(n), C.c_int(slot), C.byref(d)))
        return d.value

    def grind(self, state34, bits):
        st = np.ascontiguousarray(state34, dtype=np.uint32).copy()
        w = C.c_uint32()
        self._chk(self.L.sp1b200_grind(self.ctx, _ptr(st), C.c_uint32(bits), C.byref(w)))
        return int(w.value), st


def parse_constraint_report(w):
    w = [int(x) for x in w]
    out, p = {}, 1
    for _ in range(w[0]):
        chip, n_fail, n_listed = w[p:p + 3]; p += 3
        rows = {}
        for _ in range(n_listed):
            row, n = w[p:p + 2]; p += 2
            rows[row] = w[p:p + n]; p += n
        out[chip] = {"n_failing_rows": n_fail, "rows": rows}
    assert p == len(w), "malformed constraint report"
    return out


def parse_interaction_report(w):
    w = [int(x) for x in w]
    keys, p = [], 3
    for _ in range(w[2]):
        kind, nv = w[p:p + 2]; p += 2
        vals = w[p:p + nv]; p += nv
        net, chip, inter, row, n_chips = w[p:p + 5]; p += 5
        chips = {w[p + 2 * i]: w[p + 2 * i + 1] for i in range(n_chips)}; p += 2 * n_chips
        keys.append({"kind": kind, "values": vals, "net": net, "first": (chip, inter, row), "chips": chips})
    assert p == len(w), "malformed interaction report"
    return {"n_unbalanced": w[0] | (w[1] << 32), "keys": keys}


def verdict_name(verdict):
    return load().sp1b200_verdict_name(C.c_uint32(verdict)).decode()


class HostChallenger:

    def __init__(self, state=None):
        self.L = load()
        self.st = np.zeros(34, np.uint32)
        if state is not None:
            self.st[:] = state

    def clone(self):
        return HostChallenger(self.st.copy())

    def observe(self, vals):
        v = np.ascontiguousarray(np.atleast_1d(vals), dtype=np.uint32)
        self.L.sp1b200_challenger_observe(_ptr(self.st), _ptr(v), C.c_uint64(v.size))

    def sample(self, n=1):
        out = np.zeros(n, np.uint32)
        self.L.sp1b200_challenger_sample(_ptr(self.st), _ptr(out), C.c_uint64(n))
        return out

    def sample_bits(self, bits):
        return int(self.L.sp1b200_challenger_sample_bits(_ptr(self.st), C.c_uint32(bits)))

    def check_witness(self, bits, w):
        return bool(self.L.sp1b200_challenger_check_witness(_ptr(self.st), C.c_uint32(bits), C.c_uint32(w)))


def _wire_args(params, names, main_w, prep_w):
    p = dict(DEFAULT_CORE_PARAMS)
    p.update(params)
    n = len(names)
    return (Params(**p), C.c_uint32(n), (C.c_char_p * n)(*[s.encode() for s in names]), (C.c_uint32 * n)(*[int(x) for x in main_w]),
            (C.c_uint32 * n)(*[int(x) for x in prep_w]))


def shard_proof_to_bincode(words, names, heights, main_w, prep_w, **params):
    L = load()
    P, n, NM, MW, PW = _wire_args(params, names, main_w, prep_w)
    H = (C.c_uint64 * len(names))(*[int(h) for h in heights])
    w = np.ascontiguousarray(words, dtype=np.uint32)
    nb = C.c_uint64()
    err = L.sp1b200_shard_proof_to_bincode(C.byref(P), n, NM, H, MW, PW, _ptr(w), C.c_uint64(w.size), None, C.c_uint64(0), C.byref(nb))
    if err:
        raise Sp1B200Error(err.decode())
    out = np.empty(nb.value, np.uint8)
    err = L.sp1b200_shard_proof_to_bincode(C.byref(P), n, NM, H, MW, PW, _ptr(w), C.c_uint64(w.size), C.c_void_p(out.ctypes.data),
                                           C.c_uint64(out.size), C.byref(nb))
    if err:
        raise Sp1B200Error(err.decode())
    return out.tobytes()


def shard_proof_from_bincode(data, names, main_w, prep_w, **params):
    L = load()
    P, n, NM, MW, PW = _wire_args(params, names, main_w, prep_w)
    buf = np.frombuffer(bytes(data), np.uint8)
    H = (C.c_uint64 * max(1, len(names)))()
    nw = C.c_uint64()
    err = L.sp1b200_shard_proof_from_bincode(C.byref(P), n, NM, MW, PW, C.c_void_p(buf.ctypes.data), C.c_uint64(buf.size), H, None,
                                             C.c_uint64(0), C.byref(nw))
    if err:
        raise Sp1B200Error(err.decode())
    out = np.empty(nw.value, np.uint32)
    err = L.sp1b200_shard_proof_from_bincode(C.byref(P), n, NM, MW, PW, C.c_void_p(buf.ctypes.data), C.c_uint64(buf.size), H, _ptr(out),
                                             C.c_uint64(out.size), C.byref(nw))
    if err:
        raise Sp1B200Error(err.decode())
    return out, [int(H[i]) for i in range(len(names))]
```

Before: 65.14 million.

## Fuse first two zerocheck sumcheck rounds via 2D grid evaluation of quads

Adds a grid-mode zerocheck that, in round 0, reads each group of four rows once and evaluates every constraint on a 12-node 2D grid. It accumulates enough sums to produce both round-0 and round-1 univariate polynomials on the host. It then folds the base-field columns directly with both challenges in one kernel. This skips the separate round-0 fold and the round-1 sum pass over the intermediate extension-field buffers. It requires constraint degree at most 3 (checked at machine creation), uses more accumulators per thread and larger partial-reduction widths, and adds intricate host-side interpolation with edge handling for odd heights.

```diff
diff --git a/include/sp1b200.h b/include/sp1b200.h
--- a/include/sp1b200.h
+++ b/include/sp1b200.h
@@ -91,6 +91,8 @@
 void sp1b200_machine_free(sp1b200_ctx* ctx, sp1b200_machine* machine);
 uint32_t sp1b200_machine_num_chips(const sp1b200_machine* machine);
 uint32_t sp1b200_machine_chip_regs(const sp1b200_machine* machine, uint32_t chip);
+int sp1b200_machine_zerocheck_grid(const sp1b200_machine* machine);
+void sp1b200_ctx_set_zerocheck_grid(sp1b200_ctx* ctx, int enable);
 
 sp1b200_err sp1b200_zerocheck(sp1b200_ctx* ctx, const sp1b200_machine* machine, const uint64_t* h_heights,
                               const uint32_t* const* d_main, const uint32_t* const* d_prep, const uint32_t* h_public_values,
diff --git a/sp1_b200/csrc/ctx.cuh b/sp1_b200/csrc/ctx.cuh
--- a/sp1_b200/csrc/ctx.cuh
+++ b/sp1_b200/csrc/ctx.cuh
@@ -20,6 +20,7 @@
     uint32_t* d_T8 = nullptr;
     uint64_t launches = 0;
     bool force_generic_ntt = false;
+    bool zc_grid = true;
     std::map<std::string, float> phase_ms;
     cudaEvent_t ev0 = nullptr, ev1 = nullptr;
     uint32_t* h_mail = nullptr;
diff --git a/sp1_b200/csrc/hostcheck.cu b/sp1_b200/csrc/hostcheck.cu
--- a/sp1_b200/csrc/hostcheck.cu
+++ b/sp1_b200/csrc/hostcheck.cu
@@ -4,6 +4,7 @@
 #include "hostfield.hpp"
 #include "septic.hpp"
 #include "zc_lower.hpp"
+#include "zc_grid.cuh"
 #include <cstring>
 #include <type_traits>
 
@@ -50,6 +51,14 @@
 uint32_t sp1b200_hostcheck_rs_tw8(uint32_t* out) {
     for (uint32_t i = 0; i < rs_tw::WORDS; i++) out[i] = rs_tw::word(i / 8, (int)(i % 8));
     return rs_tw::WORDS;
+}
+void sp1b200_hostcheck_zc_grid(const uint32_t* quads, uint64_t n, uint32_t* out, int32_t* xy) {
+    for (uint64_t i = 0; i < n; i++) {
+        uint32_t v[ZC_GRID_NODES];
+        zc_grid_expand(quads[4 * i], quads[4 * i + 1], quads[4 * i + 2], quads[4 * i + 3], v);
+        for (int k = 0; k < ZC_GRID_NODES; k++) out[ZC_GRID_NODES * i + k] = v[k];
+    }
+    for (int k = 0; k < ZC_GRID_NODES; k++) { xy[2 * k] = zc_grid_x(k); xy[2 * k + 1] = zc_grid_y(k); }
 }
 void sp1b200_hostcheck_field(const uint32_t* a, const uint32_t* b, uint32_t* add, uint32_t* sub, uint32_t* mul, uint64_t n) {
     for (uint64_t i = 0; i < n; i++) { add[i] = kb::add(a[i], b[i]); sub[i] = kb::sub(a[i], b[i]); mul[i] = kb::mul(a[i], b[i]); }
diff --git a/sp1_b200/csrc/machine.cuh b/sp1_b200/csrc/machine.cuh
--- a/sp1_b200/csrc/machine.cuh
+++ b/sp1_b200/csrc/machine.cuh
@@ -66,6 +66,7 @@
     void* d_zc_arena = nullptr;
     ChipProg* d_chips = nullptr;
     void* interactions = nullptr;
+    bool zc_grid = false;
 };
 
 void* sp1b200_parse_interactions(const uint32_t* b, const uint32_t* end, size_t n_chips, const uint32_t* widths);
diff --git a/sp1_b200/csrc/zc_grid.cuh b/sp1_b200/csrc/zc_grid.cuh
--- /dev/null
+++ b/sp1_b200/csrc/zc_grid.cuh
@@ -0,0 +1,27 @@
+#pragma once
+#include "kb31.cuh"
+
+constexpr int ZC_GRID_NODES = 12;
+KB_HD constexpr int zc_grid_x(int n) { return n < 4 ? ((n & 1) ? 4 : 2) : (((n - 4) & 3) == 3 ? 4 : ((n - 4) & 3)); }
+KB_HD constexpr int zc_grid_y(int n) { return n < 2 ? 0 : n < 4 ? 1 : n < 8 ? 2 : 4; }
+
+KB_HD void zc_grid_expand(uint32_t c00, uint32_t c10, uint32_t c01, uint32_t c11, uint32_t (&v)[ZC_GRID_NODES]) {
+    using namespace kb;
+    const uint32_t b0 = sub(c10, c00), b1 = sub(c11, c01);
+    const uint32_t dy = sub(c01, c00), db = sub(b1, b0);
+    const uint32_t b0x2 = add(b0, b0), b1x2 = add(b1, b1);
+    v[0] = add(c00, b0x2);
+    v[1] = add(v[0], b0x2);
+    v[2] = add(c01, b1x2);
+    v[3] = add(v[2], b1x2);
+    const uint32_t a2 = add(c01, dy), b2 = add(b1, db);
+    v[4] = a2;
+    v[5] = add(a2, b2);
+    v[6] = add(v[5], b2);
+    v[7] = add(v[6], add(b2, b2));
+    const uint32_t a4 = add(a2, add(dy, dy)), b4 = add(b2, add(db, db));
+    v[8] = a4;
+    v[9] = add(a4, b4);
+    v[10] = add(v[9], b4);
+    v[11] = add(v[10], add(b4, b4));
+}
diff --git a/sp1_b200/csrc/zerocheck.cu b/sp1_b200/csrc/zerocheck.cu
--- a/sp1_b200/csrc/zerocheck.cu
+++ b/sp1_b200/csrc/zerocheck.cu
@@ -7,6 +7,7 @@
 #include <vector>
 
 #include "machine.cuh"
+#include "zc_grid.cuh"
 #include "zc_lower.hpp"
 #include "sumcheck.cuh"
 
@@ -230,20 +231,123 @@
     }
 }
 
+template <int RF>
+__global__ void __launch_bounds__(ZC_BLOCK) zc_sum2_kernel(const ZcJob* __restrict__ jobs, int n_jobs, const ChipProg* __restrict__ chips,
+                                                           const uint32_t* __restrict__ pv, const uint32_t* __restrict__ gkr_pows,
+                                                           const uint32_t* __restrict__ E, uint32_t* __restrict__ partial,
+                                                           void* __restrict__ ws, uint32_t ws_regs) {
+    constexpr int NN = ZC_GRID_NODES;
+    extern __shared__ __align__(16) unsigned char zc_smem[];
+    const ZcJob job = jobs[find_job(jobs, n_jobs, blockIdx.x)];
+    const ChipProg& prog = chips[job.chip];
+    const uint32_t* main = static_cast<const uint32_t*>(job.main);
+    const uint32_t* prep = static_cast<const uint32_t*>(job.prep);
+    const uint64_t h = job.h;
+    const uint64_t quads = (h + 3) / 4;
+    RegFile<uint32_t, RF, NN> rf(zc_smem, ws, ws_regs);
+    Ext acc[NN + 4];
+#pragma unroll
+    for (int a = 0; a < NN + 4; a++) acc[a] = kb::ext_zero();
+    const ZcInstr* __restrict__ zc = prog.zc + job.zc_begin;
+    const uint32_t n_zc = job.zc_end - job.zc_begin;
+    uint32_t* corners = static_cast<uint32_t*>(const_cast<void*>(job.batch));
+    auto quad = [&](const uint32_t* c, uint64_t q, uint32_t (&w)[4]) {
+        const uint64_t r = 4 * q;
+#pragma unroll
+        for (int k = 0; k < 4; k++) w[k] = r + k < h ? __ldg(c + r + k) : 0u;
+    };
+    for (uint64_t q = (uint64_t)(blockIdx.x - job.blk_start) * ZC_BLOCK + threadIdx.x; q < quads; q += (uint64_t)job.nblk * ZC_BLOCK) {
+        const Ext e = kb::ext_load(E + 4 * q);
+        const bool y1 = 4 * q + 2 < h;
+        ZcInstr in = n_zc ? zc[0] : ZcInstr{};
+        for (uint32_t pc = 0; pc < n_zc; pc++) {
+            const ZcInstr nxt = zc[pc + 1 < n_zc ? pc + 1 : pc];
+            switch (in.op) {
+                case ZC_LOAD_MAIN: case ZC_LOAD_PREP: {
+                    uint32_t w[4], v[NN];
+                    quad((in.op == ZC_LOAD_MAIN ? main : prep) + (uint64_t)((uint32_t)in.a | ((uint32_t)in.b << 16)) * h, q, w);
+                    zc_grid_expand(w[0], w[1], w[2], w[3], v);
+#pragma unroll
+                    for (int n = 0; n < NN; n++) rf.set(in.out, n, v[n]);
+                    break;
+                }
+                case ZC_CONST: case ZC_PUBLIC: {
+                    const uint32_t c = in.op == ZC_CONST ? prog.consts[in.a] : pv[prog.publics[in.a]];
+#pragma unroll
+                    for (int n = 0; n < NN; n++) rf.set(in.out, n, c);
+                    break; }
+                case ZC_ADD: {
+                    uint32_t r[NN];
+#pragma unroll
+                    for (int n = 0; n < NN; n++) r[n] = kb::add(rf.get(in.a, n), rf.get(in.b, n));
+#pragma unroll
+                    for (int n = 0; n < NN; n++) rf.set(in.out, n, r[n]);
+                    break; }
+                case ZC_SUB: {
+                    uint32_t r[NN];
+#pragma unroll
+                    for (int n = 0; n < NN; n++) r[n] = kb::sub(rf.get(in.a, n), rf.get(in.b, n));
+#pragma unroll
+                    for (int n = 0; n < NN; n++) rf.set(in.out, n, r[n]);
+                    break; }
+                case ZC_MUL: {
+                    uint32_t r[NN];
+#pragma unroll
+                    for (int n = 0; n < NN; n++) r[n] = kb::mul(rf.get(in.a, n), rf.get(in.b, n));
+#pragma unroll
+                    for (int n = 0; n < NN; n++) rf.set(in.out, n, r[n]);
+                    break; }
+                case ZC_NEG: {
+                    uint32_t r[NN];
+#pragma unroll
+                    for (int n = 0; n < NN; n++) r[n] = kb::sub(0u, rf.get(in.a, n));
+#pragma unroll
+                    for (int n = 0; n < NN; n++) rf.set(in.out, n, r[n]);
+                    break; }
+                case ZC_ASSERT: {
+                    const Ext al = kb::ext_load(job.alpha_pows + 4 * in.b);
+                    const Ext ae = kb::ext_mul(al, e);
+#pragma unroll
+                    for (int n = 0; n < NN; n++)
+                        if (zc_grid_y(n) != 1 || y1) acc[n] = kb::ext_add(acc[n], kb::ext_mul_base(ae, rf.get(in.a, n)));
+                    break; }
+                default: __trap();
+            }
+            in = nxt;
+        }
+        if (!job.columns) continue;
+        Ext s[4] = {kb::ext_zero(), kb::ext_zero(), kb::ext_zero(), kb::ext_zero()};
+        for (uint32_t j = 0; j < prog.main_w + prog.prep_w; j++) {
+            const Ext g = kb::ext_load(gkr_pows + 4 * j);
+            uint32_t w[4];
+            quad(j < prog.main_w ? main + (uint64_t)j * h : prep + (uint64_t)(j - prog.main_w) * h, q, w);
+#pragma unroll
+            for (int k = 0; k < 4; k++) s[k] = kb::ext_add(s[k], kb::ext_mul_base(g, w[k]));
+        }
+#pragma unroll
+        for (int k = 0; k < 4; k++) {
+            acc[NN + k] = kb::ext_add(acc[NN + k], kb::ext_mul(s[k], e));
+            if (corners) kb::ext_store(corners + 16 * q + 4 * k, s[k]);
+        }
+    }
+    block_reduce<NN + 4>(acc, partial, Mail{nullptr, nullptr, 0});
+}
+
+template <int W>
 __global__ void __launch_bounds__(128) zc_reduce_kernel(const ZcJob* __restrict__ jobs, const uint32_t* __restrict__ partial, uint32_t* __restrict__ out,
                                                         Mail mail) {
     const ZcJob job = jobs[blockIdx.x];
-    __shared__ uint32_t red[36][4];
+    __shared__ uint32_t red[W][4];
     const int slot = threadIdx.x >> 2, part = threadIdx.x & 3;
-    for (int w = slot; w < 36; w += 32) {
+    for (int w = slot; w < W; w += 32) {
         uint32_t v = 0;
-        for (uint32_t b = part; b < job.nblk; b += 4) v = kb::add(v, partial[(uint64_t)(job.blk_start + b) * 36 + w]);
+        for (uint32_t b = part; b < job.nblk; b += 4) v = kb::add(v, partial[(uint64_t)(job.blk_start + b) * W + w]);
         red[w][part] = v;
     }
     __syncthreads();
-    if (threadIdx.x < 36) {
+    if (threadIdx.x < W) {
         const uint32_t* r = red[threadIdx.x];
-        out[blockIdx.x * 36 + threadIdx.x] = kb::add(kb::add(r[0], r[1]), kb::add(r[2], r[3]));
+        out[blockIdx.x * W + threadIdx.x] = kb::add(kb::add(r[0], r[1]), kb::add(r[2], r[3]));
     }
     sp1_mail_done(mail);
 }
@@ -266,6 +370,36 @@
     if constexpr (sizeof(K) == 4) r = kb::ext_add(kb::ext_from_base(a), kb::ext_mul_base(alpha, kb::sub(b, a)));
     else r = kb::ext_add(a, kb::ext_mul(alpha, kb::ext_sub(b, a)));
     kb::ext_store(job.out + 4 * t, r);
+}
+
+__global__ void __launch_bounds__(256) zc_fix2_kernel(const ZcFixJob* __restrict__ jobs, int n_jobs, Ext a0, Ext a1) {
+    const ZcFixJob job = jobs[find_job(jobs, n_jobs, blockIdx.x)];
+    const uint64_t h = job.h, nq = (h + 3) / 4;
+    const uint32_t bpc = (uint32_t)((nq + 255) / 256);
+    const uint32_t lb = blockIdx.x - job.blk_start;
+    const uint64_t j = lb / bpc;
+    const uint64_t q = (uint64_t)(lb - (uint32_t)j * bpc) * 256 + threadIdx.x;
+    if (q >= nq) return;
+    const uint32_t* in = j < job.main_w ? static_cast<const uint32_t*>(job.main) + j * h
+                                        : static_cast<const uint32_t*>(job.prep) + (j - job.main_w) * h;
+    uint32_t w[4];
+#pragma unroll
+    for (int k = 0; k < 4; k++) w[k] = 4 * q + k < h ? __ldg(in + 4 * q + k) : 0u;
+    const Ext r0 = kb::ext_add(kb::ext_from_base(w[0]), kb::ext_mul_base(a0, kb::sub(w[1], w[0])));
+    const Ext r1 = kb::ext_add(kb::ext_from_base(w[2]), kb::ext_mul_base(a0, kb::sub(w[3], w[2])));
+    kb::ext_store(job.out + 4 * (j * nq + q), kb::ext_add(r0, kb::ext_mul(a1, kb::ext_sub(r1, r0))));
+}
+
+__global__ void __launch_bounds__(256) zc_batch2_kernel(const ZcFixJob* __restrict__ jobs, int n_jobs, Ext a0, Ext a1) {
+    const ZcFixJob job = jobs[find_job(jobs, n_jobs, blockIdx.x)];
+    const uint64_t nq = (job.h + 3) / 4;
+    const uint64_t q = (uint64_t)(blockIdx.x - job.blk_start) * 256 + threadIdx.x;
+    if (q >= nq) return;
+    const uint32_t* s = static_cast<const uint32_t*>(job.main) + 16 * q;
+    const Ext s00 = kb::ext_load(s), s10 = kb::ext_load(s + 4), s01 = kb::ext_load(s + 8), s11 = kb::ext_load(s + 12);
+    const Ext r0 = kb::ext_add(s00, kb::ext_mul(a0, kb::ext_sub(s10, s00)));
+    const Ext r1 = kb::ext_add(s01, kb::ext_mul(a0, kb::ext_sub(s11, s01)));
+    kb::ext_store(job.out + 4 * q, kb::ext_add(r0, kb::ext_mul(a1, kb::ext_sub(r1, r0))));
 }
 
 __global__ void __launch_bounds__(256) zc_batch0_kernel(const ZcFixJob* __restrict__ jobs, int n_jobs, const uint32_t* __restrict__ gkr_pows, Ext alpha) {
@@ -432,6 +566,23 @@
         m->interactions = sp1b200_parse_interactions(b, end, n, widths.data());
         if (!m->interactions) return sp1b200_last_error();
     }
+    {
+        m->zc_grid = true;
+        for (uint32_t c = 0; c < n && m->zc_grid; c++) {
+            const HostProg& hp = m->host[c];
+            std::vector<uint32_t> deg(std::max<uint32_t>(m->chips[c].n_regs, 1), 0);
+            for (const DagInstr& in : hp.instrs) {
+                switch (in.opcode) {
+                    case BC_LOAD_LEAF: deg[in.out] = 1; break;
+                    case BC_LOAD_CONST: case BC_LOAD_PUBLIC: deg[in.out] = 0; break;
+                    case BC_ADD_F: case BC_SUB_F: deg[in.out] = std::max(deg[in.a], deg[in.b]); break;
+                    case BC_MUL_F: deg[in.out] = std::min<uint32_t>(deg[in.a] + deg[in.b], 1u << 16); break;
+                    case BC_NEG_F: deg[in.out] = deg[in.a]; break;
+                }
+            }
+            for (uint32_t r : hp.assert_regs) if (deg[r] > 3) m->zc_grid = false;
+        }
+    }
     std::vector<ZcInstr> all;
     std::vector<size_t> zc_off(n);
     for (uint32_t c = 0; c < n; c++) {
@@ -465,6 +616,8 @@
 void sp1b200_machine_free(sp1b200_ctx*, sp1b200_machine* m) { delete m; }
 uint32_t sp1b200_machine_chip_regs(const sp1b200_machine* m, uint32_t chip) { return chip < m->chips.size() ? m->chips[chip].zc_regs : 0; }
 uint32_t sp1b200_machine_num_chips(const sp1b200_machine* m) { return (uint32_t)m->chips.size(); }
+int sp1b200_machine_zerocheck_grid(const sp1b200_machine* m) { return m->zc_grid ? 1 : 0; }
+void sp1b200_ctx_set_zerocheck_grid(sp1b200_ctx* ctx, int enable) { ctx->zc_grid = enable != 0; }
 
 sp1b200_err sp1b200_zerocheck(sp1b200_ctx* ctx, const sp1b200_machine* m, const uint64_t* h_heights, const uint32_t* const* d_main,
                               const uint32_t* const* d_prep, const uint32_t* h_pv, uint32_t n_pv, const uint32_t* h_gkr_point,
@@ -475,6 +628,7 @@
     for (size_t k = 0; k < nchips; k++)
         for (uint32_t pi : m->host[k].publics)
             if (pi >= n_pv) return sp1b200_set_error("zerocheck: chip %zu reads public value %u but only %u were passed", k, pi, n_pv);
+    const bool grid = mlr >= 2 && m->zc_grid && ctx->zc_grid;
     cudaStream_t st = ctx->stream;
     DevFree mem(ctx);
     HostChallenger ch;
@@ -485,7 +639,7 @@
     const E4 alpha = E4::load(h_alpha), gamma = E4::load(h_gamma);
 
     struct St {
-        uint64_t h;
+        uint64_t h, h0;
         std::vector<E4> zeta; E4 eq_adj = E4::one(), pra; VGeq vg;
     };
     std::vector<St> S(nchips);
@@ -507,12 +661,13 @@
     for (uint32_t i = 0; i < mlr; i++) gp[i] = E4::load(h_gkr_point + 4 * i);
     std::vector<E4> all_ap; all_ap.reserve(total_c);
     std::vector<size_t> ap_off(nchips), woff(nchips);
-    std::vector<uint64_t> boff0(nchips), boff1(nchips);
+    std::vector<uint64_t> boff0(nchips), boff1(nchips), coff(nchips);
+    uint64_t c_words = 0;
     uint64_t b0 = 0, b1 = 0; size_t wsum = 0;
     for (size_t k = 0; k < nchips; k++) {
         const ChipProg& p = m->chips[k];
         St& s = S[k];
-        s.h = h_heights[k];
+        s.h = s.h0 = h_heights[k];
         if (s.h > ((uint64_t)1 << mlr)) return sp1b200_set_error("zerocheck: chip %zu height exceeds 2^%u", k, mlr);
         if (p.zc_regs > ZC_GLOBAL_REGS) return sp1b200_set_error("zerocheck: chip %zu needs %u live registers (> %d)", k, p.zc_regs, ZC_GLOBAL_REGS);
         s.zeta = gp;
@@ -525,9 +680,11 @@
         s.vg.threshold = (uint32_t)s.h; s.vg.geq_c = E4::one();
         const uint64_t nh = (s.h + 1) / 2;
         const size_t w = p.main_w + p.prep_w;
-        boff0[k] = b0; b0 += (uint64_t)(w + 1) * nh * 4;
+        const uint64_t n_odd = grid ? (((nh + 1) / 2) + 1) / 2 : nh;
+        boff0[k] = b0; b0 += (uint64_t)(w + 1) * n_odd * 4;
         boff1[k] = b1; b1 += (uint64_t)(w + 1) * ((nh + 1) / 2) * 4;
         woff[k] = wsum; wsum += w;
+        if (grid) { coff[k] = c_words; c_words += 16 * ((s.h + 3) / 4); }
     }
     SP1_TRY(mem.alloc((void**)&d_ap, all_ap.size() * 16));
     SP1_CUDA(cudaMemcpyAsync(d_ap, all_ap.data(), all_ap.size() * 16, cudaMemcpyHostToDevice, st));
@@ -535,6 +692,8 @@
     SP1_TRY(mem.alloc((void**)&d_buf[0], b0 * 4 + 16));
     SP1_TRY(mem.alloc((void**)&d_buf[1], b1 * 4 + 16));
     SP1_TRY(mem.alloc((void**)&d_final, (wsum ? wsum : 1) * 16));
+    uint32_t* d_corners = nullptr;
+    if (c_words) SP1_TRY(mem.alloc((void**)&d_corners, c_words * 4));
     uint32_t *d_point, *d_E[2];
     SP1_TRY(mem.alloc((void**)&d_point, mlr * 16));
     SP1_CUDA(cudaMemcpyAsync(d_point, h_gkr_point, mlr * 16, cudaMemcpyHostToDevice, st));
@@ -551,7 +710,7 @@
     std::vector<ZcFixJob> fjobs, bjobs;
     uint32_t batch_blocks = 0;
     const unsigned MAXB = 132 * 4;
-    uint32_t max_blocks = 1, max_jobs = 1;
+    uint32_t max_blocks = 36, max_jobs = 1;
     {
         std::vector<uint64_t> hcur(nchips);
         for (size_t k = 0; k < nchips; k++) hcur[k] = S[k].h;
@@ -568,17 +727,18 @@
                 return static_cast<const uint32_t*>(in_main(k)) + (uint64_t)p.main_w * hcur[k] * 4;
             };
             auto in_batch = [&](size_t k) -> const void* {
-                if (rd == 0) return nullptr;
+                if (rd == 0) return grid ? d_corners + coff[k] : nullptr;
                 const ChipProg& p = m->chips[k];
                 return static_cast<const uint32_t*>(in_main(k)) + (uint64_t)(p.main_w + p.prep_w) * hcur[k] * 4;
             };
             uint32_t blocks_round = 0;
-            for (int tier = 0; tier < 5; tier++) {
+            const bool sum2 = grid && rd == 0;
+            for (int tier = 0; tier < 5 && !(grid && rd == 1); tier++) {
                 Launch Lc{jobs.size(), 0, 0, 0, tier};
                 for (size_t k = 0; k < nchips; k++) {
                     const ChipProg& p = m->chips[k];
                     if (!hcur[k] || zc_tier(p.zc_regs) != tier) continue;
-                    unsigned nb = blocks_for((hcur[k] + 1) / 2, ZC_BLOCK);
+                    unsigned nb = blocks_for(sum2 ? (hcur[k] + 3) / 4 : (hcur[k] + 1) / 2, ZC_BLOCK);
                     if (nb > MAXB) nb = MAXB;
                     if (tier == 4 && nb > ZC_GLOBAL_MAXB) nb = ZC_GLOBAL_MAXB;
                     const auto& pieces = m->host[k].zc_pieces;
@@ -603,7 +763,7 @@
                     if (tier == 4) ws_bytes = std::max(ws_bytes, (size_t)Lc.blocks * Lc.regs * 3 * ZC_BLOCK * 16);
                 }
             }
-            max_blocks = std::max(max_blocks, blocks_round);
+            max_blocks = std::max(max_blocks, blocks_round * (sum2 ? 64u : 36u));
             max_jobs = std::max<uint32_t>(max_jobs, (uint32_t)R.chip_of_job.size());
             R.fix0 = fjobs.size(); R.fix_jobs = 0; R.fix_blocks = 0;
             for (size_t k = 0; k < nchips; k++) {
@@ -611,6 +771,19 @@
                 if (!hcur[k]) continue;
                 const uint64_t nh = (hcur[k] + 1) / 2;
                 uint32_t* out = rd + 1 == mlr ? d_final + 4 * woff[k] : (rd & 1 ? d_buf[1] + boff1[k] : d_buf[0] + boff0[k]);
+                if (grid && rd == 0) { hcur[k] = nh; continue; }
+                if (grid && rd == 1) {
+                    const void* prep = p.prep_w ? d_prep[k] : nullptr;
+                    fjobs.push_back(ZcFixJob{d_main[k], prep, out, S[k].h, p.main_w, p.prep_w, R.fix_blocks, 0});
+                    R.fix_jobs++; R.fix_blocks += blocks_for(nh, 256) * (p.main_w + p.prep_w);
+                    if (rd + 1 < mlr) {
+                        bjobs.push_back(ZcFixJob{d_corners + coff[k], nullptr, out + (uint64_t)(p.main_w + p.prep_w) * nh * 4, S[k].h, 0, 0,
+                                                 batch_blocks, 0});
+                        batch_blocks += blocks_for(nh, 256);
+                    }
+                    hcur[k] = nh;
+                    continue;
+                }
                 const uint32_t fold_b = (rd > 0 && rd + 1 < mlr) ? 1u : 0u;
                 ZcFixJob f{in_main(k), in_prep(k), out, hcur[k], p.main_w, p.prep_w + fold_b, R.fix_blocks, 0};
                 fjobs.push_back(f);
@@ -632,8 +805,8 @@
     if (!bjobs.empty()) SP1_CUDA(cudaMemcpyAsync(d_bjobs, bjobs.data(), bjobs.size() * sizeof(ZcFixJob), cudaMemcpyHostToDevice, st));
     if (!jobs.empty()) SP1_CUDA(cudaMemcpyAsync(d_jobs, jobs.data(), jobs.size() * sizeof(ZcJob), cudaMemcpyHostToDevice, st));
     if (!fjobs.empty()) SP1_CUDA(cudaMemcpyAsync(d_fjobs, fjobs.data(), fjobs.size() * sizeof(ZcFixJob), cudaMemcpyHostToDevice, st));
-    SP1_TRY(mem.alloc((void**)&d_partial, (size_t)max_blocks * 36 * 4));
-    if ((size_t)max_jobs * 36 > SP1_MAIL_WORDS) return sp1b200_set_error("zerocheck: %u chips exceed the mailbox payload", max_jobs);
+    SP1_TRY(mem.alloc((void**)&d_partial, (size_t)max_blocks * 4));
+    if ((size_t)max_jobs * 64 > SP1_MAIL_WORDS) return sp1b200_set_error("zerocheck: %u chips exceed the mailbox payload", max_jobs);
     d_sums = sp1b200_mail_dev(ctx);
     SP1_CUDA(cudaMemsetAsync(d_final, 0, (wsum ? wsum : 1) * 16, st));
     void* d_ws = nullptr;
@@ -650,6 +823,17 @@
         const size_t regs = Lc.regs;
         return ext ? go(zc_sum_kernel<Ext, RF_SMEM, false>, regs * 3 * ZC_BLOCK * 16) : go(zc_sum_kernel<uint32_t, RF_SMEM, true>, regs * 3 * ZC_BLOCK * 4);
     };
+    auto launch_sum2 = [&](const Launch& Lc, uint32_t* part) -> sp1b200_err {
+        auto go = [&](auto kern, size_t smem) -> sp1b200_err {
+            if (smem > 32 * 1024) SP1_CUDA(cudaFuncSetAttribute(kern, cudaFuncAttributeMaxDynamicSharedMemorySize, (int)smem));
+            SP1_LAUNCH(ctx, kern, Lc.blocks, ZC_BLOCK, smem, d_jobs + Lc.job0, (int)Lc.n_jobs, m->d_chips, d_pv, d_gw, d_E[1], part, d_ws,
+                       Lc.regs);
+            return nullptr;
+        };
+        if (Lc.tier == 4) return go(zc_sum2_kernel<RF_GLOBAL>, 0);
+        if (Lc.tier == 3) return go(zc_sum2_kernel<RF_LOCAL>, 0);
+        return go(zc_sum2_kernel<RF_SMEM>, (size_t)Lc.regs * ZC_GRID_NODES * ZC_BLOCK * 4);
+    };
 
     t_setup.reset();
     E4 lambda; ch.sample_ext(lambda.c);
@@ -660,29 +844,75 @@
     words.push_back(mlr);
     std::vector<E4> point;
     std::vector<E4> ys((size_t)nchips * 4);
-    std::vector<uint32_t> hs((size_t)max_jobs * 36);
+    std::vector<uint32_t> hs((size_t)max_jobs * 64);
     std::vector<E4> chip_sums(nchips * 9);
+    std::vector<E4> grid_sums(grid ? nchips * 16 : 0);
+    auto eq_entry = [](const std::vector<E4>& z, size_t k, uint64_t idx) {
+        E4 r = E4::one();
+        for (size_t t = 0; t < k; t++) r = r * (((idx >> (k - 1 - t)) & 1) ? z[t] : E4::one() - z[t]);
+        return r;
+    };
     const E4 two = E4::from_base(hf::to_monty(2)), four = E4::from_base(hf::to_monty(4)), three = E4::from_base(hf::to_monty(3));
     for (uint32_t rd = 0; rd < mlr; rd++) {
         const RoundPlan& R = plan[rd];
+        const bool sum2 = grid && rd == 0;
+        const uint32_t W = sum2 ? 64 : 36;
+        if (sum2) SP1_TRY(launch_halve_eq(ctx, d_E[0], (uint64_t)1 << (mlr - 2), d_E[1]));
         {
             uint32_t blk = 0, seq = 0; size_t jb = 0;
             for (const Launch& Lc : R.sums) {
-                SP1_TRY(launch_sum(Lc, rd > 0, d_partial + (size_t)blk * 36));
+                SP1_TRY(sum2 ? launch_sum2(Lc, d_partial + (size_t)blk * W) : launch_sum(Lc, rd > 0, d_partial + (size_t)blk * W));
                 const Mail mail = sp1b200_mail_next(ctx); seq = mail.seq;
-                SP1_LAUNCH(ctx, zc_reduce_kernel, Lc.n_jobs, 128, 0, d_jobs + Lc.job0, d_partial + (size_t)blk * 36, d_sums + jb * 36, mail);
+                if (sum2) SP1_LAUNCH(ctx, zc_reduce_kernel<64>, Lc.n_jobs, 128, 0, d_jobs + Lc.job0, d_partial + (size_t)blk * W, d_sums + jb * W, mail);
+                else SP1_LAUNCH(ctx, zc_reduce_kernel<36>, Lc.n_jobs, 128, 0, d_jobs + Lc.job0, d_partial + (size_t)blk * W, d_sums + jb * W, mail);
                 blk += Lc.blocks; jb += Lc.n_jobs;
             }
             if (jb) {
                 HostSpan sp(acc_wait);
                 SP1_TRY(sp1b200_mail_wait(ctx, seq));
-                memcpy(hs.data(), sp1b200_mail_host(ctx), jb * 36 * 4);
+                memcpy(hs.data(), sp1b200_mail_host(ctx), jb * W * 4);
             }
         }
         HostSpan sp_math(acc_math);
         std::fill(chip_sums.begin(), chip_sums.end(), E4());
-        for (size_t j = 0; j < R.chip_of_job.size(); j++)
-            for (int w9 = 0; w9 < 9; w9++) chip_sums[(size_t)R.chip_of_job[j] * 9 + w9] = chip_sums[(size_t)R.chip_of_job[j] * 9 + w9] + E4::load(&hs[j * 36 + 4 * w9]);
+        if (sum2) {
+            std::fill(grid_sums.begin(), grid_sums.end(), E4());
+            for (size_t j = 0; j < R.chip_of_job.size(); j++)
+                for (int w = 0; w < 16; w++) grid_sums[(size_t)R.chip_of_job[j] * 16 + w] = grid_sums[(size_t)R.chip_of_job[j] * 16 + w] + E4::load(&hs[j * 64 + 4 * w]);
+        } else if (!grid || rd != 1) {
+            for (size_t j = 0; j < R.chip_of_job.size(); j++)
+                for (int w9 = 0; w9 < 9; w9++) chip_sums[(size_t)R.chip_of_job[j] * 9 + w9] = chip_sums[(size_t)R.chip_of_job[j] * 9 + w9] + E4::load(&hs[j * 36 + 4 * w9]);
+        }
+        if (grid && rd <= 1) {
+            const E4 z = gp[mlr - 2], a0 = rd == 1 ? point[0] : E4();
+            E4 L[4];
+            if (rd == 1) {
+                const E4 xs[4] = {E4(), E4::one(), two, four};
+                E4 basis4[4][4];
+                hf::lagrange_basis<4>(xs, basis4);
+                for (int i = 0; i < 4; i++) L[i] = hf::eval_poly<4>(basis4[i], a0);
+            }
+            for (size_t k = 0; k < nchips; k++) {
+                const E4* G = &grid_sums[k * 16];
+                const E4 *T = G, *C = G + 12;
+                E4* q = &chip_sums[k * 9];
+                if (rd == 0) {
+                    const E4 z0 = E4::one() - z;
+                    q[1] = z0 * C[0] + z * C[2];
+                    q[2] = z0 * C[1] + z * C[3];
+                    q[3] = z0 * T[0] + z * T[2];
+                    q[6] = z0 * T[1] + z * T[3];
+                } else {
+                    const E4 b0 = E4::one() - a0;
+                    q[0] = L[2] * T[0] + L[3] * T[1];
+                    if (S[k].h0 % 4 == 1) q[0] = q[0] + L[1] * S[k].pra * eq_entry(S[k].zeta, S[k].zeta.size() - 1, (S[k].h0 - 1) / 4);
+                    q[3] = L[0] * T[4] + L[1] * T[5] + L[2] * T[6] + L[3] * T[7];
+                    q[6] = L[0] * T[8] + L[1] * T[9] + L[2] * T[10] + L[3] * T[11];
+                    q[1] = b0 * C[0] + a0 * C[1];
+                    q[2] = b0 * C[2] + a0 * C[3];
+                }
+            }
+        }
         const E4 last = gp[mlr - 1 - rd];
         const E4 bnode = (E4::one() - last) * hf::inv(E4::one() - (last + last));
         const E4 nodes[5] = {E4(), E4::one(), two, four, bnode};
@@ -725,7 +955,12 @@
         E4 a; ch.sample_ext(a.c);
         point.insert(point.begin(), a);
         const Ext da = to_ext(a);
-        if (R.fix_jobs) {
+        if (grid && rd == 1) {
+            const Ext d0 = to_ext(point[1]);
+            if (R.fix_jobs) SP1_LAUNCH(ctx, zc_fix2_kernel, R.fix_blocks, 256, 0, d_fjobs + R.fix0, (int)R.fix_jobs, d0, da);
+            if (!bjobs.empty()) SP1_LAUNCH(ctx, zc_batch2_kernel, batch_blocks, 256, 0, d_bjobs, (int)bjobs.size(), d0, da);
+        } else if (grid && rd == 0) {
+        } else if (R.fix_jobs) {
             if (rd == 0) {
                 SP1_LAUNCH(ctx, zc_fix_kernel<uint32_t>, R.fix_blocks, 256, 0, d_fjobs + R.fix0, (int)R.fix_jobs, da);
                 if (!bjobs.empty()) SP1_LAUNCH(ctx, zc_batch0_kernel, batch_blocks, 256, 0, d_bjobs, (int)bjobs.size(), d_gw, da);
@@ -743,7 +978,8 @@
             s.zeta.pop_back();
             s.h = (s.h + 1) / 2;
         }
-        if (rd + 1 < mlr) {
+        if (grid && rd == 0) ecur = 1;
+        else if (rd + 1 < mlr) {
             const uint64_t n_out = (uint64_t)1 << (mlr - 2 - rd);
             SP1_TRY(launch_halve_eq(ctx, d_E[ecur], n_out, d_E[ecur ^ 1]));
             ecur ^= 1;
diff --git a/sp1_b200/lib.py b/sp1_b200/lib.py
--- a/sp1_b200/lib.py
+++ b/sp1_b200/lib.py
@@ -56,6 +56,7 @@
         L.sp1b200_challenger_check_witness.restype = C.c_int
         L.sp1b200_machine_num_chips.restype = C.c_uint32
         L.sp1b200_machine_chip_regs.restype = C.c_uint32
+        L.sp1b200_machine_zerocheck_grid.restype = C.c_int
         L.sp1b200_verdict_name.restype = C.c_char_p
         for name in ERR_FUNCS:
             getattr(L, name).restype = C.c_char_p
@@ -74,7 +75,8 @@
 OTHER_FUNCS = ["sp1b200_challenger_init", "sp1b200_challenger_observe", "sp1b200_challenger_sample",
                "sp1b200_challenger_sample_bits", "sp1b200_challenger_check_witness", "sp1b200_ctx_destroy", "sp1b200_default_core_params", "sp1b200_version", "sp1b200_ctx_stream",
                "sp1b200_launch_count", "sp1b200_last_phase_ms", "sp1b200_commit_free", "sp1b200_jagged_round_free",
-               "sp1b200_machine_free", "sp1b200_machine_num_chips", "sp1b200_machine_chip_regs",
+               "sp1b200_machine_free", "sp1b200_machine_num_chips", "sp1b200_machine_chip_regs", "sp1b200_machine_zerocheck_grid",
+               "sp1b200_ctx_set_zerocheck_grid",
                "sp1b200_verdict_name"]
 
 
@@ -216,6 +218,12 @@
 
     def machine_chip_regs(self, h, chip):
         return int(self.L.sp1b200_machine_chip_regs(h, C.c_uint32(chip)))
+
+    def machine_zerocheck_grid(self, h):
+        return bool(self.L.sp1b200_machine_zerocheck_grid(h))
+
+    def set_zerocheck_grid(self, enable):
+        self.L.sp1b200_ctx_set_zerocheck_grid(self.ctx, C.c_int(1 if enable else 0))
 
     def machine_free(self, h):
         self.L.sp1b200_machine_free(self.ctx, h)
```

New measurement: 67.06 million (median of 6 runs). 1.03x the previous value.
